# vision-agh/apse_uav

Hardware: AMD Instinct MI355X
Metric: 4K UAV frames/sec (whole node) (higher is better)
Workload: dtype f32

## Files before the change

apse_uav_amd/_lib.py:

```python
import ctypes as C
import os

import numpy as np

_HERE = os.path.dirname(os.path.abspath(__file__))
_TREE_LIB = os.path.join(_HERE, "libapse_hip.so")
LIB_PATH = os.environ.get("APSE_HIP_LIB") or _TREE_LIB
TOOL_ENTRIES = ("apse_winograd_pack_filter", "apse_winograd_conv2d")

APSE_OK = 0


class ApseError(RuntimeError):
    pass


class Config(C.Structure):
    _fields_ = [
        ("struct_size", C.c_int), ("device", C.c_int), ("max_batch", C.c_int),
        ("frame_h", C.c_int), ("frame_w", C.c_int), ("image_h", C.c_int), ("image_w", C.c_int),
        ("blocks", C.c_int * 4), ("num_classes", C.c_int),
        ("score_thresh", C.c_float), ("box_nms", C.c_float), ("rpn_nms", C.c_float), ("mask_thresh", C.c_float),
        ("rpn_pre_topk", C.c_int), ("rpn_post_topk", C.c_int), ("dets_per_image", C.c_int),
        ("pixel_mean", C.c_float * 3), ("assoc_roi", C.c_int), ("embed_dim", C.c_int), ("assoc_scale", C.c_float),
        ("compute_dtype", C.c_int), ("storage16", C.c_int),
    ]


class ConfigArch(Config):
    _fields_ = [("arch", C.c_int)]


class ResultsLayout(C.Structure):
    _fields_ = [("bytes", C.c_size_t), ("n_max", C.c_int), ("dets_per_image", C.c_int), ("embed_dim", C.c_int),
                ("max_batch", C.c_int)] + [(k, C.c_size_t) for k in (
                    "total", "offset", "prop_count", "img", "cls", "roi", "score", "box_resized", "box", "valid", "rect",
                    "mass", "centroid", "closest", "embedding")]


class RenderItem(C.Structure):
    _fields_ = [("image", C.c_int), ("rect", C.c_int * 4), ("words_per_row", C.c_int), ("bits", C.c_void_p),
                ("box", C.c_float * 4), ("rgb", C.c_uint8 * 4), ("label_off", C.c_int), ("label_len", C.c_int)]


class MotsWindow(C.Structure):
    _fields_ = [("rect", C.c_int * 4), ("words_per_row", C.c_int), ("area", C.c_int), ("bits", C.c_void_p)]


class MotsObject(C.Structure):
    _fields_ = [("rect", C.c_int * 4), ("words_per_row", C.c_int), ("score", C.c_float), ("bits", C.c_void_p)]


class ConvDesc(C.Structure):
    _fields_ = [(k, C.c_int) for k in ("B", "H", "W", "Cin", "Cout", "KH", "KW", "stride", "pad", "relu", "res_mode",
                                       "cfg", "splitk", "prec", "fuse_reduce", "x_st", "res_st", "y_st")]


_lib = None


def load():
    global _lib
    if _lib is not None:
        return _lib
    if not os.path.exists(LIB_PATH):
        raise ApseError("libapse_hip.so not found at %s: build it with `python -c 'import __graft_entry__ as g; g.build()'` "
                        "or `make -C apse_uav_amd/csrc` (there is no CPU fallback)" % LIB_PATH)
    import torch
    lib = C.CDLL(LIB_PATH)
    vp, i, f, sz = C.c_void_p, C.c_int, C.c_float, C.c_size_t
    sig = {
        "apse_create": ([C.POINTER(Config), C.POINTER(vp)], i),
        "apse_destroy": ([vp], None),
        "apse_last_error": ([vp], C.c_char_p),
        "apse_version": ([], C.c_char_p),
        "apse_set_weight": ([vp, C.c_char_p, vp, C.POINTER(C.c_int64), i], i),
        "apse_finalize_weights": ([vp], i),
        "apse_set_resize_tables": ([vp, vp, vp, i, vp, vp, i], i),
        "apse_set_camera": ([vp, C.POINTER(C.c_double), C.POINTER(C.c_double), i, vp, i, i], i),
        "apse_preprocess_frames": ([vp, vp, i, vp], i),
        "apse_preprocess_images": ([vp, vp, i, vp], i),
        "apse_backbone": ([vp, i, vp], i),
        "apse_rpn": ([vp, i, vp], i),
        "apse_rpn_levels": ([vp, i, i, vp], i),
        "apse_box_head": ([vp, i, vp], i),
        "apse_set_detections": ([vp, vp, vp, vp, vp, i, vp], i),
        "apse_mask_tail": ([vp, i, vp], i),
        "apse_embed": ([vp, i, vp], i),
        "apse_forward": ([vp, i, vp], i),
        "apse_results_describe": ([vp, C.POINTER(ResultsLayout)], i),
        "apse_read_results": ([vp, vp, sz, vp], i),
        "apse_read_results_begin": ([vp, vp, sz, vp], i),
        "apse_read_results_end": ([vp, vp], i),
        "apse_copy_mask_window": ([vp, i, i, i, i, i, vp, vp], i),
        "apse_copy_mask_windows": ([vp, i, vp, vp, vp, vp, vp], i),
        "apse_host_copy": ([vp, vp, sz, i], i),
        "apse_feature_shape": ([vp, C.c_char_p, C.POINTER(C.c_int * 3)], i),
        "apse_export_feature": ([vp, C.c_char_p, vp, i, vp], i),
        "apse_debug_tensor": ([vp, C.c_char_p, vp, sz, C.POINTER(sz), vp], i),
        "apse_flops": ([vp, i, C.c_double, C.c_double], C.c_double),
        "apse_profile": ([vp, i], i),
        "apse_profile_read": ([vp, C.POINTER(C.c_double * 42), i], i),
        "apse_conv_packed_elems": ([C.POINTER(ConvDesc)], sz),
        "apse_conv_pack_weight": ([C.POINTER(ConvDesc), vp, i, vp, vp], i),
        "apse_conv2d": ([C.POINTER(ConvDesc), vp, vp, vp, vp, vp, vp, sz, vp], i),
        "apse_winograd_pack_filter": ([vp, i, i, vp], i),
        "apse_winograd_conv2d": ([C.POINTER(ConvDesc), vp, vp, vp, vp, vp], i),
        "apse_maxpool3x3s2": ([vp, vp, i, i, i, i, vp], i),
        "apse_maxpool3x3s2_typed": ([vp, vp, i, i, i, i, i, vp], i),
        "apse_roi_align": ([C.POINTER(vp), C.POINTER(i), C.POINTER(i), vp, i, i, i, vp, vp], i),
        "apse_roi_align_typed": ([C.POINTER(vp), C.POINTER(i), C.POINTER(i), vp, i, i, i, i, vp, vp], i),
        "apse_roi_pool": ([vp, i, i, vp, vp, i, i, f, vp, vp], i),
        "apse_roi_features": ([vp, i, vp, vp, i, i, vp, vp], i),
        "apse_nms_rank": ([vp, vp, vp, i, i, i, i, f, i, vp, vp, vp, vp, vp], i),
        "apse_mask_centroid_dense": ([vp, i, i, C.POINTER(C.c_int * 3), vp], i),
        "apse_mask_closest_dense": ([vp, i, i, f, f, C.POINTER(C.c_int * 2), vp], i),
        "apse_l2_normalize": ([vp, vp, i, i, vp], i),
        "apse_sqdist": ([vp, vp, i, i, i, vp, vp], i),
        "apse_undistort_gamma": ([vp, vp, i, i, i, C.POINTER(C.c_double), C.POINTER(C.c_double), i, vp, i, i, vp], i),
        "apse_lab_tables_host": ([vp, vp, C.c_size_t], C.c_size_t),
        "apse_replay_create": ([i, i, f, i], vp),
        "apse_replay_destroy": ([vp], None),
        "apse_replay_step": ([vp, i, i, vp, vp, vp, C.c_char_p, i, vp], i),
        "apse_replay_packed": ([vp, vp, C.c_longlong, i, i, i, vp, C.c_longlong], C.c_longlong),
        "apse_replay_max_id": ([vp], i),
        "apse_replay_next_id": ([vp], i),
        "apse_render_workspace_bytes": ([i, i, i], sz),
        "apse_render_instances": ([vp, vp, i, i, i, i, vp, i, vp, sz, vp, i, vp, sz, vp], i),
        "apse_render_pack_mask": ([vp, i, i, vp, vp], i),
        "apse_render_font_host": ([vp, sz], sz),
        "apse_mots_split_workspace_bytes": ([], sz),
        "apse_mots_split_idmap": ([vp, i, i, i, vp, sz, vp, vp, vp, vp, sz, vp], i),
        "apse_mots_rle_to_bits": ([vp, vp, i, i, i, vp, vp], i),
        "apse_mots_overlaps": ([vp, i, vp, i, vp, i, vp, vp], i),
        "apse_mots_shift_overlaps": ([vp, i, vp, i, i, i, vp, vp], i),
        "apse_mots_render_idmap": ([vp, vp, i, i, i, vp, vp], i),
        "apse_resize_normalize": ([vp, vp, vp, vp, vp, vp, i, vp, vp, i, i, i, i, i, i, i, i, C.POINTER(f * 3), vp], i),
        "apse_assoc_fc_workspace_bytes": ([i, i, i], sz),
        "apse_assoc_fc_forward": ([vp, vp, vp, i, i, i, vp, vp, vp, sz, vp], i),
        "apse_assoc_fc_backward": ([vp, vp, vp, vp, i, i, i, vp, vp, vp, sz, vp], i),
        "apse_triplet_workspace_bytes": ([i], sz),
        "apse_triplet_hard_forward": ([vp, vp, i, i, f, i, vp, vp, sz, vp], i),
        "apse_triplet_all_forward": ([vp, vp, i, i, f, i, vp, vp, sz, vp], i),
        "apse_triplet_hard_backward": ([vp, i, i, i, vp, vp, vp, vp], i),
        "apse_triplet_all_backward": ([vp, i, i, i, vp, vp, vp, vp], i),
        "apse_sgd_step": ([vp, vp, vp, C.c_longlong, f, f, f, f, i, i, vp], i),
        "apse_coco_box_iou": ([vp, vp, vp, i, i, i, vp, vp, vp, vp, vp], i),
        "apse_coco_poly_to_bits": ([vp, vp, i, vp, i, vp, vp, vp, i, vp, vp, vp, vp], i),
        "apse_coco_match": ([vp, vp, vp, i, i, i, vp, vp, vp, i, vp, vp, vp, i, vp, i, vp, i, vp, vp, vp, vp, vp], i),
        "apse_coco_accumulate_workspace_bytes": ([C.c_longlong], sz),
        "apse_coco_sort_lists": ([vp, vp, i, vp, C.c_longlong, i, vp, vp, sz, vp], i),
        "apse_coco_accumulate": ([vp, vp, vp, i, vp, i, vp, vp, vp, C.c_longlong, i, vp, i, i, i, i, i, vp, vp, vp, vp, sz,
                                  vp], i),
        "apse_mask_roi_features": ([vp, i, vp, i, vp, vp], i),
        "apse_mask_train_workspace_bytes": ([i, i], sz),
        "apse_mask_pack_elems": ([i, i, i, i], sz),
        "apse_mask_pack_weight": ([vp, vp, i, i, i, i, i, vp, vp, vp], i),
        "apse_mask_conv_forward": ([vp, vp, vp, i, i, i, i, i, i, i, i, i, i, i, vp, vp, sz, vp], i),
        "apse_mask_conv3x3": ([vp, vp, vp, i, i, vp, vp], i),
        "apse_mask_relu_grad": ([vp, vp, C.c_longlong, vp, vp], i),
        "apse_mask_bias_grad": ([vp, C.c_longlong, vp, vp, sz, vp], i),
        "apse_mask_wgrad": ([vp, vp, i, i, vp, vp, sz, vp], i),
        "apse_mask_loss_forward": ([vp, i, vp, vp, i, vp, vp, sz, vp], i),
        "apse_mask_loss_backward": ([vp, i, vp, vp, i, vp, vp, vp], i),
        "apse_mask_predictor_backward": ([vp, vp, vp, vp, i, i, vp, vp, vp, vp, sz, vp], i),
        "apse_augment_u8": ([vp, i, i, i, vp, vp, vp, vp, vp], i),
    }
    for name, (args, ret) in sig.items():
        if name in TOOL_ENTRIES and LIB_PATH != _TREE_LIB and not hasattr(lib, name):
            continue
        fn = getattr(lib, name)
        fn.argtypes = args
        fn.restype = ret
    _lib = lib
    return lib


EXPORTS = ["apse_create", "apse_destroy", "apse_last_error", "apse_version", "apse_set_weight", "apse_finalize_weights",
           "apse_set_resize_tables", "apse_set_camera", "apse_preprocess_frames", "apse_preprocess_images", "apse_backbone", "apse_rpn", "apse_rpn_levels",
           "apse_box_head", "apse_set_detections", "apse_mask_tail", "apse_embed", "apse_forward", "apse_results_describe",
           "apse_read_results", "apse_read_results_begin", "apse_read_results_end", "apse_copy_mask_window", "apse_copy_mask_windows", "apse_host_copy", "apse_feature_shape", "apse_export_feature", "apse_debug_tensor",
           "apse_flops", "apse_profile", "apse_profile_read", "apse_conv_packed_elems", "apse_conv_pack_weight", "apse_conv2d", "apse_winograd_pack_filter", "apse_winograd_conv2d", "apse_maxpool3x3s2",
           "apse_maxpool3x3s2_typed", "apse_roi_align", "apse_roi_align_typed", "apse_roi_pool", "apse_roi_features", "apse_nms_rank", "apse_mask_centroid_dense", "apse_mask_closest_dense",
           "apse_l2_normalize", "apse_sqdist", "apse_undistort_gamma", "apse_lab_tables_host", "apse_resize_normalize", "apse_replay_create", "apse_replay_destroy",
           "apse_replay_step", "apse_replay_packed", "apse_replay_max_id", "apse_replay_next_id", "apse_render_workspace_bytes",
           "apse_render_instances", "apse_render_pack_mask", "apse_render_font_host", "apse_mots_split_workspace_bytes",
           "apse_mots_split_idmap", "apse_mots_rle_to_bits", "apse_mots_overlaps", "apse_mots_shift_overlaps", "apse_mots_render_idmap",
           "apse_assoc_fc_workspace_bytes", "apse_assoc_fc_forward", "apse_assoc_fc_backward", "apse_triplet_workspace_bytes",
           "apse_triplet_hard_forward", "apse_triplet_all_forward", "apse_triplet_hard_backward", "apse_triplet_all_backward",
           "apse_sgd_step", "apse_coco_box_iou", "apse_coco_poly_to_bits", "apse_coco_match",
           "apse_coco_accumulate_workspace_bytes", "apse_coco_sort_lists", "apse_coco_accumulate",
           "apse_mask_roi_features", "apse_mask_train_workspace_bytes", "apse_mask_pack_elems", "apse_mask_pack_weight",
           "apse_mask_conv_forward", "apse_mask_conv3x3", "apse_mask_relu_grad", "apse_mask_bias_grad", "apse_mask_wgrad", "apse_mask_loss_forward",
           "apse_mask_loss_backward", "apse_mask_predictor_backward", "apse_augment_u8"]


def stream_ptr():
    import torch
    return C.c_void_p(torch.cuda.current_stream().cuda_stream)


def check(rc, ctx=None, what=""):
    if rc != APSE_OK:
        msg = load().apse_last_error(ctx).decode() if ctx is not None else ""
        raise ApseError("%s failed (code %d) %s" % (what, rc, msg))


def ptr(t):
    if t is None:
        return C.c_void_p(0)
    if isinstance(t, np.ndarray):
        assert t.flags["C_CONTIGUOUS"]
        return C.c_void_p(t.ctypes.data)
    assert t.is_contiguous()
    return C.c_void_p(t.data_ptr())
```

apse_uav_amd/config.py:

```python
import copy
import os

import yaml


class CfgNode(dict):
    def __init__(self, init=None):
        super().__init__()
        self.__dict__["_frozen"] = False
        for k, v in (init or {}).items():
            self[k] = CfgNode(v) if isinstance(v, dict) else v

    def __getattr__(self, k):
        try:
            return self[k]
        except KeyError:
            raise AttributeError(k)

    def __setattr__(self, k, v):
        if self.__dict__.get("_frozen"):
            raise AttributeError("attempt to modify frozen CfgNode key %r" % k)
        self[k] = v

    def freeze(self):
        self.__dict__["_frozen"] = True
        for v in self.values():
            if isinstance(v, CfgNode):
                v.freeze()

    def defrost(self):
        self.__dict__["_frozen"] = False
        for v in self.values():
            if isinstance(v, CfgNode):
                v.defrost()

    def clone(self):
        c = CfgNode(copy.deepcopy(_plain(self)))
        return c

    def _merge(self, other):
        for k, v in other.items():
            if isinstance(v, dict) and isinstance(self.get(k), CfgNode):
                self[k]._merge(v)
            else:
                self[k] = CfgNode(v) if isinstance(v, dict) else (tuple(v) if isinstance(v, list) else v)

    def merge_from_file(self, path):
        data = _load_yaml_chain(path)
        if (data.get("MODEL", {}).get("ROI_HEADS", {}).get("NAME") == C4_ROI_HEADS and "MODEL" in self
                and not is_c4(self)):
            _apply_c4_defaults(self)
        self._merge(data)

    def merge_from_list(self, kv):
        for k, v in zip(kv[0::2], kv[1::2]):
            node = self
            parts = k.split(".")
            for p in parts[:-1]:
                node = node[p]
            node[parts[-1]] = v


def _deep_update(dst, src):
    for k, v in src.items():
        if isinstance(v, dict) and isinstance(dst.get(k), dict):
            _deep_update(dst[k], v)
        else:
            dst[k] = v
    return dst


def _load_yaml_chain(path):
    with open(path) as f:
        data = yaml.safe_load(f) or {}
    base = data.pop("_BASE_", None)
    if not base:
        return data
    if not os.path.isabs(base):
        base = os.path.join(os.path.dirname(path), base)
    return _deep_update(_load_yaml_chain(base), data)


def _plain(n):
    return {k: (_plain(v) if isinstance(v, CfgNode) else v) for k, v in n.items()}


def get_cfg():
    return CfgNode({
        "VERSION": 2,
        "MODEL": {
            "DEVICE": "cuda",
            "META_ARCHITECTURE": "GeneralizedRCNN",
            "WEIGHTS": "",
            "MASK_ON": True,
            "PIXEL_MEAN": (103.530, 116.280, 123.675),
            "PIXEL_STD": (1.0, 1.0, 1.0),
            "BACKBONE": {"NAME": "build_resnet_fpn_backbone"},
            "RESNETS": {"DEPTH": 101, "OUT_FEATURES": ("res2", "res3", "res4", "res5"),
                        "STRIDE_IN_1X1": True, "NORM": "FrozenBN", "RES2_OUT_CHANNELS": 256, "STEM_OUT_CHANNELS": 64},
            "FPN": {"IN_FEATURES": ("res2", "res3", "res4", "res5"), "OUT_CHANNELS": 256, "FUSE_TYPE": "sum", "NORM": ""},
            "ANCHOR_GENERATOR": {"SIZES": ((32,), (64,), (128,), (256,), (512,)),
                                 "ASPECT_RATIOS": ((0.5, 1.0, 2.0),), "OFFSET": 0.0},
            "RPN": {"IN_FEATURES": ("p2", "p3", "p4", "p5", "p6"), "PRE_NMS_TOPK_TEST": 1000,
                    "POST_NMS_TOPK_TEST": 1000, "NMS_THRESH": 0.7, "BBOX_REG_WEIGHTS": (1.0, 1.0, 1.0, 1.0),
                    "MIN_SIZE": 0},
            "ROI_HEADS": {"NAME": "StandardROIHeads", "IN_FEATURES": ("p2", "p3", "p4", "p5"), "NUM_CLASSES": 80,
                          "SCORE_THRESH_TEST": 0.05, "NMS_THRESH_TEST": 0.5},
            "ROI_BOX_HEAD": {"NAME": "FastRCNNConvFCHead", "NUM_FC": 2, "FC_DIM": 1024, "POOLER_RESOLUTION": 7,
                             "POOLER_SAMPLING_RATIO": 0, "POOLER_TYPE": "ROIAlignV2",
                             "BBOX_REG_WEIGHTS": (10.0, 10.0, 5.0, 5.0)},
            "ROI_MASK_HEAD": {"NAME": "MaskRCNNConvUpsampleHead", "NUM_CONV": 4, "CONV_DIM": 256,
                              "POOLER_RESOLUTION": 14, "POOLER_SAMPLING_RATIO": 0, "POOLER_TYPE": "ROIAlignV2"},
        },
        "INPUT": {"MIN_SIZE_TEST": 800, "MAX_SIZE_TEST": 1333, "FORMAT": "BGR", "MIN_SIZE_TRAIN": (800,), "MAX_SIZE_TRAIN": 1333,
                  "MIN_SIZE_TRAIN_SAMPLING": "choice"},
        "TEST": {"DETECTIONS_PER_IMAGE": 100},
        "DATASETS": {"TRAIN": ("coco_2017_train",), "TEST": ("coco_2017_val",)},
        "APSE": {"DTYPE": "f32", "MAX_BATCH": 1, "FUSED_PREPROC": True, "STORAGE16": True, "CONTEXT_CACHE": 1},
    })


C4_ROI_HEADS = "Res5ROIHeads"
C4_ANCHOR_SIZES = ((32, 64, 128, 256, 512),)
C4_ANCHOR_RATIOS = ((0.5, 1.0, 2.0),)


def is_c4(cfg):
    return cfg.MODEL.ROI_HEADS.NAME == C4_ROI_HEADS


def _apply_c4_defaults(cfg):
    m = cfg.MODEL
    m.BACKBONE.NAME = "build_resnet_backbone"
    m.RESNETS.OUT_FEATURES = ("res4",)
    m.RESNETS.RES5_DILATION = 1
    m.ANCHOR_GENERATOR.SIZES = C4_ANCHOR_SIZES
    m.ANCHOR_GENERATOR.ASPECT_RATIOS = C4_ANCHOR_RATIOS
    m.RPN.IN_FEATURES = ("res4",)
    m.RPN.PRE_NMS_TOPK_TEST = 6000
    m.RPN.POST_NMS_TOPK_TEST = 1000
    m.ROI_HEADS.NAME = C4_ROI_HEADS
    m.ROI_HEADS.IN_FEATURES = ("res4",)
    m.ROI_BOX_HEAD.NAME = ""
    m.ROI_BOX_HEAD.NUM_FC = 0
    m.ROI_BOX_HEAD.POOLER_RESOLUTION = 14
    m.ROI_MASK_HEAD.NUM_CONV = 0
    m.ROI_MASK_HEAD.POOLER_RESOLUTION = 14


def check_c4_supported(cfg):
    m = cfg.MODEL
    if tuple(tuple(s) for s in m.ANCHOR_GENERATOR.SIZES) != C4_ANCHOR_SIZES or \
            tuple(tuple(r) for r in m.ANCHOR_GENERATOR.ASPECT_RATIOS) != C4_ANCHOR_RATIOS or \
            float(m.ANCHOR_GENERATOR.get("OFFSET", 0.0)) != 0.0:
        raise ValueError("C4: only detectron2's default anchors are supported (sizes %s, ratios %s, offset 0)"
                         % (C4_ANCHOR_SIZES, C4_ANCHOR_RATIOS))
    if int(m.RESNETS.get("RES5_DILATION", 1)) != 1:
        raise ValueError("C4: RES5_DILATION 2 is not supported")
    if not m.MASK_ON:
        raise ValueError("C4: box-only models (MASK_ON False) are not supported")
    if tuple(m.RPN.IN_FEATURES) != ("res4",) or tuple(m.ROI_HEADS.IN_FEATURES) != ("res4",):
        raise ValueError("C4: the RPN and the ROI heads read res4")
    if int(m.ROI_BOX_HEAD.POOLER_RESOLUTION) != 14 or int(m.ROI_MASK_HEAD.POOLER_RESOLUTION) != 14 or \
            int(m.ROI_MASK_HEAD.NUM_CONV) != 0:
        raise ValueError("C4: pooler resolution 14 and no mask convolutions (NUM_CONV 0) are required")


CLASSES_NAMES = ["car", "truck", "bus", "person"]


def setup_cfg(weights="", score_thresh=0.5, num_classes=4, device="cuda", arch="FPN"):
    if arch not in ("FPN", "C4"):
        raise ValueError("arch must be 'FPN' or 'C4'")
    cfg = get_cfg()
    if arch == "C4":
        _apply_c4_defaults(cfg)
    cfg.MODEL.ROI_HEADS.SCORE_THRESH_TEST = score_thresh
    cfg.MODEL.ROI_HEADS.NUM_CLASSES = num_classes
    cfg.MODEL.WEIGHTS = weights
    cfg.MODEL.MASK_ON = True
    cfg.MODEL.DEVICE = device
    return cfg
```

apse_uav_amd/csrc/detector.hip:

```cpp
#include "detector_ctx.h"

#include <math.h>
#include <string.h>

static std::string g_create_error;

int fail(apse_ctx* c, int code, const std::string& msg) {
    if (c) c->err = msg; else g_create_error = msg;
    return code;
}
int apse_fail_global(int code, const char* msg) { return fail(nullptr, code, msg); }

static int take_event_pair(apse_ctx* c, hipStream_t s) {
    if (!c->prof_on) return -1;
    if (c->ev_used == 0) {
        hipEventRecord(c->ev_pool[c->ev_base], s);
        hipEventRecord(c->ev_pool[c->ev_base + 1], s);
        c->ev_used = 2;
    }
    if (c->ev_used + 2 > APSE_EV_HALF) return -1;
    const int e0 = c->ev_base + c->ev_used;
    c->ev_used += 2;
    return e0;
}

static int run_plan(apse_ctx* c, std::vector<Step>& plan, int batch, hipStream_t s) {
    int* total_dev = reinterpret_cast<int*>(c->res + c->lay.total);
    int* propcnt_dev = reinterpret_cast<int*>(c->res + c->lay.prop_count);
    for (size_t si = 0; si < plan.size(); ++si) {
        Step& st = plan[si];
        int rc = APSE_OK;
        if (st.kind == S_CONV) {
            ConvParams p = st.c.p;
            for (size_t sj = si + 1; sj < plan.size() && sj <= si + 2; ++sj)
                if (plan[sj].kind == S_CONV) {
                    const ConvParams& q = plan[sj].c.p;
                    const size_t elems = q.wu ? (size_t)16 * q.Cout * (1 << q.cin_log2) : (size_t)apse_roundup(q.Cout, 128) * q.KH * q.KWCp;
                    p.next_w = q.w16 ? (const void*)q.w16 : (q.wu ? (const void*)q.wu : (const void*)q.w);
                    const size_t bytes = elems * (q.w16 ? 2 : 4);
                    p.next_w_bytes = bytes > (64u << 20) ? (64u << 20) : (unsigned)bytes;
                    break;
                }
            p.B = st.c.fixed_items > 0 ? st.c.fixed_items : batch * st.c.b_mult;
            p.M = p.B * p.OH * p.OW;
            p.ws = c->ws;
            p.tile_cnt = nullptr;
            p.m_count = nullptr; p.m_per_item = p.OH * p.OW; p.m_hint = 0;
            int cfg = st.c.cfg;
            if (st.c.count_kind == 2) {
                p.m_count = total_dev;
                const int mh = (c->hint_total > 0 ? c->hint_total : 1) * p.m_per_item;
                p.m_hint = mh < p.M ? mh : p.M;
                if (p.prec != 0 && p.splitk == 1 && (cfg == 0 || cfg == 1 || cfg == 3)) {
                    int sk_dyn = 1;
                    const int cfg_dyn = apse_conv_pick_cfg(p.m_hint, p.Cout, p.steps_total, &sk_dyn);
                    if (sk_dyn == 1 && (cfg_dyn == 0 || cfg_dyn == 1 || cfg_dyn == 3)) cfg = cfg_dyn;
                }
            }
            else if (st.c.count_kind == 1 && batch == 1) p.m_count = propcnt_dev;
            const int e0 = take_event_pair(c, s);
            const hipEvent_t ev0 = e0 >= 0 ? c->ev_pool[e0] : nullptr, ev1 = e0 >= 0 ? c->ev_pool[e0 + 1] : nullptr;
            if (st.c.pool_y) {
                rc = apse_k_stem_pool16(p.x, p.w16, p.bias, st.c.pool_y, batch, p.H, p.W, p.prec, s, ev0, ev1);
                cfg = APSE_CFG_STEMPOOL;
            } else if (p.wu) {
                rc = apse_launch_conv_winograd(p, s, ev0, ev1);
            } else {
                rc = apse_launch_conv(p, cfg, s, ev0, ev1);
                cfg = apse_conv_effective_cfg(p, cfg);
            }
            if (e0 >= 0) c->pending.push_back({cfg, st.c.flops_per_item, st.c.count_kind, st.c.b_mult, batch, e0, e0 + 1});
        } else if (st.kind == S_BNECK) {
            const int e0 = take_event_pair(c, s);
            const ConvParams& q1 = st.c.p;
            rc = apse_k_bottleneck64_fused16(st.x, st.p3.res, st.y, q1.w16, q1.bias, st.p2.w16, st.p2.bias, st.p3.w16, st.p3.bias, batch,
                                             st.H, st.W, st.C, st.st, s, e0 >= 0 ? c->ev_pool[e0] : nullptr,
                                             e0 >= 0 ? c->ev_pool[e0 + 1] : nullptr);
            if (e0 >= 0) c->pending.push_back({APSE_CFG_BNECK, st.c.flops_per_item, 0, 1, batch, e0, e0 + 1});
        } else if (st.kind == S_MAXPOOL) {
            rc = apse_k_maxpool3x3s2(st.x, st.y, batch, st.H, st.W, st.C, st.st, s);
        } else {
            rc = apse_k_subsample2(st.x, st.y, batch, st.H, st.W, st.C, st.st, s);
        }
        if (rc != APSE_OK) return fail(c, rc, "launch failed at step " + st.c.name);
    }
    return APSE_OK;
}

int fill_camera(UndistortParams& p, int H, int W, const double* m, const double* dist, int ndist, int do_undistort, int do_gamma) {
    memset(&p, 0, sizeof p);
    if (!m || ndist > 14 || ndist < 0 || (ndist > 0 && !dist)) return APSE_E_INVALID;
    for (int i = 0; i < ndist && i < 12; ++i) p.k[i] = dist[i];
    if (ndist > 12 && (dist[12] != 0.0 || (ndist > 13 && dist[13] != 0.0))) return APSE_E_INVALID;
    const double a = m[0], b = m[1], c = m[2], dd = m[3], e = m[4], f = m[5], g = m[6], h = m[7], k = m[8];
    const double det = a * (e * k - f * h) - b * (dd * k - f * g) + c * (dd * h - e * g);
    if (det == 0.0) return APSE_E_INVALID;
    const double id = 1.0 / det;
    p.ir[0] = (e * k - f * h) * id; p.ir[1] = (c * h - b * k) * id; p.ir[2] = (b * f - c * e) * id;
    p.ir[3] = (f * g - dd * k) * id; p.ir[4] = (a * k - c * g) * id; p.ir[5] = (c * dd - a * f) * id;
    p.ir[6] = (dd * h - e * g) * id; p.ir[7] = (b * g - a * h) * id; p.ir[8] = (a * e - b * dd) * id;
    p.fx = m[0]; p.fy = m[4]; p.u0 = m[2]; p.v0 = m[5];
    p.H = H; p.W = W; p.do_undistort = do_undistort; p.do_gamma = do_gamma;
    return APSE_OK;
}

extern "C" {

#ifndef APSE_SRC_HASH
#define APSE_SRC_HASH "unknown"
#endif
const char* apse_version(void) { return "apse_hip 0.6 (gfx950, f32 / bf16 / f16 MFMA) src " APSE_SRC_HASH; }

int apse_create(const apse_config* cfg, apse_ctx** out) {
    if (!cfg || !out) return fail(nullptr, APSE_E_INVALID, "null argument");
    const int old_size = (int)offsetof(apse_config, arch);
    if (cfg->struct_size != (int)sizeof(apse_config) && cfg->struct_size != old_size)
        return fail(nullptr, APSE_E_INVALID, "apse_config size mismatch");
    apse_config cf;
    memset(&cf, 0, sizeof cf);
    memcpy(&cf, cfg, (size_t)cfg->struct_size);
    cf.struct_size = (int)sizeof(apse_config);
    cfg = &cf;
    if (cfg->arch != 0 && cfg->arch != 1) return fail(nullptr, APSE_E_INVALID, "arch must be 0 (FPN) or 1 (C4)");
    if (cfg->arch == 1) {
        if (cfg->rpn_pre_topk < 1 || cfg->rpn_pre_topk > APSE_C4_MAX_PRE_TOPK)
            return fail(nullptr, APSE_E_INVALID, "C4 (arch 1): rpn_pre_topk " + std::to_string(cfg->rpn_pre_topk) + " outside 1.." +
                                                 std::to_string(APSE_C4_MAX_PRE_TOPK));
        if (cfg->compute_dtype != 0)
            return fail(nullptr, APSE_E_INVALID, "C4 (arch 1): compute_dtype must be 0 (f32); the 16-bit modes are FPN only");
        if (cfg->max_batch > APSE_C4_MAX_BATCH)
            return fail(nullptr, APSE_E_INVALID, "C4 (arch 1): max_batch " + std::to_string(cfg->max_batch) + " above the limit " +
                                                 std::to_string(APSE_C4_MAX_BATCH));
    }
    const int pre_cap = cfg->arch == 1 ? APSE_C4_MAX_PRE_TOPK : 1000;
    if (cfg->max_batch < 1 || cfg->max_batch > 64 || cfg->rpn_pre_topk > pre_cap || cfg->rpn_post_topk > 1000 ||
        cfg->dets_per_image > 100 || cfg->num_classes < 1 || cfg->num_classes > APSE_MAX_CLASSES || cfg->embed_dim > 256 ||
        cfg->max_batch * cfg->dets_per_image > 1024)
        return fail(nullptr, APSE_E_INVALID, "config out of supported range");
    {
        const double t = cfg->score_thresh;
        const double per_roi = t > 0.0 ? ceil(1.0 / t) - 1.0 : (double)cfg->num_classes;
        const double bound = (double)cfg->rpn_post_topk * (per_roi < cfg->num_classes ? per_roi : (double)cfg->num_classes);
        if (bound >= 40000.0)
            return fail(nullptr, APSE_E_INVALID,
                        "box candidate bound rpn_post_topk * min(num_classes, ceil(1 / score_thresh) - 1) = " +
                            std::to_string((long long)bound) + " reaches 40000, where detectron2's batched_nms changes method");
    }
    if (cfg->frame_h < 1 || cfg->frame_w < 1 || cfg->frame_h > APSE_MAX_FRAME_H || cfg->frame_w > APSE_MAX_FRAME_W)
        return fail(nullptr, APSE_E_INVALID, "frame size out of supported range (1 <= frame_h <= " + std::to_string(APSE_MAX_FRAME_H) +
                                             ", 1 <= frame_w <= " + std::to_string(APSE_MAX_FRAME_W) + ")");
    if (cfg->compute_dtype < 0 || cfg->compute_dtype > 2 || (cfg->compute_dtype && !cfg->storage16))
        return fail(nullptr, APSE_E_INVALID, "compute_dtype 1 / 2 (bf16 / f16 matrix cores) needs storage16 = 1: the f32-storage variant "
                                             "of the 16-bit modes was removed in round 4 (no BASELINE configuration uses it)");
    int ndev = 0;
    if (hipGetDeviceCount(&ndev) != hipSuccess || ndev <= 0)
        return fail(nullptr, APSE_E_HIP, "no HIP device visible: the apse_uav hot path has no CPU fallback");
    if (hipSetDevice(cfg->device) != hipSuccess) return fail(nullptr, APSE_E_HIP, "hipSetDevice failed");
    apse_ctx* c = new apse_ctx();
    c->cfg = *cfg;
    c->c4 = cfg->arch == 1;
    {
        const char* e = getenv("APSE_F32_WINOGRAD");
        c->f32_winograd = !(e && atoi(e) == 0);
    }
    *out = c;
    return APSE_OK;
}

void apse_destroy(apse_ctx* c) {
    if (!c) return;
    hipSetDevice(c->cfg.device);
    for (void* p : c->allocs) hipFree(p);
    if (c->rf_mask) hipFree(c->rf_mask);
    if (c->mrf_idx) hipFree(c->mrf_idx);
    if (c->read_ev) hipEventDestroy(c->read_ev);
    for (int k = 0; k < 2; ++k) {
        if (c->given_ev[k]) hipEventDestroy(c->given_ev[k]);
        if (c->given_host[k]) hipHostFree(c->given_host[k]);
    }
    delete c;
}

const char* apse_last_error(apse_ctx* c) { return c ? c->err.c_str() : g_create_error.c_str(); }

int apse_set_weight(apse_ctx* c, const char* name, const float* host, const int64_t* shape, int ndim) {
    if (!c || !name || !host || !shape || ndim < 1 || ndim > 4) return fail(c, APSE_E_INVALID, "bad weight argument");
    if (c->finalized) return fail(c, APSE_E_STATE, "weights already finalized");
    HostW w;
    size_t n = 1;
    for (int i = 0; i < ndim; ++i) { w.shape.push_back(shape[i]); n *= (size_t)shape[i]; }
    w.v.assign(host, host + n);
    c->hw[name] = std::move(w);
    return APSE_OK;
}

int apse_finalize_weights(apse_ctx* c) {
    if (!c) return APSE_E_INVALID;
    if (c->finalized) return fail(c, APSE_E_STATE, "already finalized");
    hipSetDevice(c->cfg.device);
    int rc = c->c4 ? build_plan_c4(c) : build_plan(c);
    if (rc) return rc;
    c->hw.clear();
    c->finalized = true;
    return APSE_OK;
}

int apse_set_resize_tables(apse_ctx* c, const int* hb, const int* hc, int hk, const int* vb, const int* vc, int vk) {
    if (!c || !hb || !hc || !vb || !vc) return fail(c, APSE_E_INVALID, "null table");
    const apse_config& g = c->cfg;
    std::vector<int> a(hb, hb + 2 * g.image_w), b(hc, hc + (size_t)hk * g.image_w), d(vb, vb + 2 * g.image_h),
        e(vc, vc + (size_t)vk * g.image_h);
    for (int i = 0; i < g.image_w; ++i)
        if (a[2 * i] < 0 || a[2 * i + 1] > hk || a[2 * i] + a[2 * i + 1] > g.frame_w) return fail(c, APSE_E_INVALID, "bad horizontal bounds");
    for (int i = 0; i < g.image_h; ++i)
        if (d[2 * i] < 0 || d[2 * i + 1] > vk || d[2 * i] + d[2 * i + 1] > g.frame_h) return fail(c, APSE_E_INVALID, "bad vertical bounds");
    c->hb = dupload(c, a); c->hc = dupload(c, b); c->vb = dupload(c, d); c->vc = dupload(c, e);
    c->hk = hk; c->vk = vk;
    c->hcT = nullptr;
    if (hk <= 8) {
        std::vector<int> t((size_t)8 * g.image_w, 0);
        for (int i = 0; i < g.image_w; ++i)
            for (int j = 0; j < a[2 * i + 1] && j < hk; ++j) t[(size_t)j * g.image_w + i] = b[(size_t)i * hk + j];
        c->hcT = dupload(c, t);
    }
    return APSE_OK;
}

#define NEED_READY(c, batch)                                                                     \
    if (!(c) || !(c)->finalized) return fail(c, APSE_E_STATE, "weights not finalized");          \
    if ((batch) < 1 || (batch) > (c)->cfg.max_batch) return fail(c, APSE_E_INVALID, "batch out of range");

int apse_preprocess_frames(apse_ctx* c, const uint8_t* frames, int batch, void* stream) {
    NEED_READY(c, batch);
    if (!c->hb) return fail(c, APSE_E_STATE, "resize tables not set");
    const apse_config& g = c->cfg;
    int rc = apse_k_pil_resize(frames, c->rs_tmp, c->t["input"].p, c->t["input"].st, nullptr, c->hb, c->hc, c->hk, c->vb, c->vc, c->vk, batch,
                               g.frame_h, g.frame_w, g.image_h, g.image_w, c->PH, c->PW, g.pixel_mean, c->cam_on ? &c->cam : nullptr, c->cam_lut, c->cam_map_ok ? c->cam_map : nullptr,
                               c->hcT, c->rs_pitch, (hipStream_t)stream);
    return rc ? fail(c, rc, "pil resize launch failed") : APSE_OK;
}

int apse_preprocess_images(apse_ctx* c, const float* images, int batch, void* stream) {
    NEED_READY(c, batch);
    const apse_config& g = c->cfg;
    int rc = apse_k_chw_norm(images, c->t["input"].p, c->t["input"].st, batch, g.image_h, g.image_w, c->PH, c->PW, g.pixel_mean,
                             (hipStream_t)stream);
    return rc ? fail(c, rc, "chw normalise launch failed") : APSE_OK;
}

int apse_backbone(apse_ctx* c, int batch, void* stream) {
    NEED_READY(c, batch);
    return run_plan(c, c->backbone, batch, (hipStream_t)stream);
}

int apse_rpn_levels(apse_ctx* c, int batch, int level_mask, void* stream) {
    NEED_READY(c, batch);
    level_mask &= 31;
    if (!level_mask) return fail(c, APSE_E_INVALID, "empty RPN level mask");
    int first_level = 0;
    while (!((level_mask >> first_level) & 1)) ++first_level;
    hipStream_t s = (hipStream_t)stream;
    const apse_config& g = c->cfg;
    if (c->c4 && level_mask != 31) return fail(c, APSE_E_INVALID, "C4 (arch 1) has one RPN level: level_mask must be 31");
    int rc = run_plan(c, c->rpnhead, batch, s);
    if (rc) return rc;
    if (c->c4) {
        int* propcnt = reinterpret_cast<int*>(c->res + c->lay.prop_count);
        rc = apse_k_c4_rpn(&c->c4r, g.rpn_pre_topk, g.rpn_post_topk, (float)g.image_h, (float)g.image_w, (float)log(1000.0 / 16.0),
                           g.rpn_nms, c->dec_boxes, c->dec_scores, c->dec_valid, c->c4_nms, c->props, c->prop_scores, c->prop_entry,
                           propcnt, batch, s);
        c->box_maxc_clean = false;
        return rc ? fail(c, rc, "C4 rpn selection launch failed") : APSE_OK;
    }
    for (size_t i = 0; i < c->stages.size(); ++i) {
        rc = apse_k_rpn_topk_stage(c->rl_dev, c->stage_dev[i], (int)c->stages[i].size(), c->lists, c->nslots, batch,
                                   i == 0 ? c->maxc : nullptr, s);
        if (rc) return fail(c, rc, "rpn top-k stage launch failed");
    }
    rc = apse_k_rpn_decode(c->rl_dev, g.rpn_pre_topk, c->lists, c->nslots, c->final_slot_dev, (float)g.image_h, (float)g.image_w,
                           (float)log(1000.0 / 16.0), c->dec_boxes, c->dec_scores, c->dec_valid, c->maxc, level_mask, batch, s);
    if (rc) return fail(c, rc, "rpn decode launch failed");
    rc = apse_k_nms_percat(c->dec_boxes, c->dec_scores, c->dec_valid, 5 * g.rpn_pre_topk, g.rpn_pre_topk, 0, c->maxc, g.rpn_nms,
                           c->keep_idx, c->keep_cnt, 5, c->nms_scratch, first_level, batch, 1, s);
    if (rc) return fail(c, rc, "rpn nms launch failed");
    int* propcnt = reinterpret_cast<int*>(c->res + c->lay.prop_count);
    rc = apse_k_rank_final(c->dec_boxes, c->dec_scores, 5 * g.rpn_pre_topk, c->keep_idx, c->keep_cnt, 5, g.rpn_post_topk, c->props,
                           c->prop_scores, c->prop_entry, propcnt, c->maxc + g.max_batch, batch, s);
    c->box_maxc_clean = true;
    if (rc) return fail(c, rc, "rpn rank launch failed");
    return APSE_OK;
}

int apse_rpn(apse_ctx* c, int batch, void* stream) { return apse_rpn_levels(c, batch, 31, stream); }

static int pack_from_dets(apse_ctx* c, int batch, hipStream_t s) {
    const apse_config& g = c->cfg;
    uint8_t* r = c->res;
    c->sums_dirty = false;
    return apse_k_pack_detections(c->det_boxes, c->det_scores, c->det_entry, c->det_cnt, batch, g.dets_per_image, g.num_classes,
                                  (float*)(r + c->lay.box_resized), (float*)(r + c->lay.score), (int*)(r + c->lay.cls),
                                  (int*)(r + c->lay.img), (int*)(r + c->lay.roi), (int*)(r + c->lay.total),
                                  (int*)(r + c->lay.offset), c->sums, s);
}

int apse_box_head(apse_ctx* c, int batch, void* stream) {
    NEED_READY(c, batch);
    hipStream_t s = (hipStream_t)stream;
    const apse_config& g = c->cfg;
    int* propcnt = reinterpret_cast<int*>(c->res + c->lay.prop_count);
    const int P = g.rpn_post_topk, K = g.num_classes;
    int rc;
    if (c->c4) {
        const Tens& f = c->t["res4"];
        rc = apse_k_roi_align_c4(f.p, f.H, f.W, f.C, 1.0f / 16.0f, c->props, nullptr, propcnt, nullptr, P, batch * P, 14,
                                 c->t["box_pooled"].p, s);
        if (rc) return fail(c, rc, "C4 roi_align(14) launch failed");
        rc = run_plan(c, c->c4_res5box, batch, s);
        if (rc) return rc;
        const Tens& r5 = c->t["box_res5"];
        rc = apse_k_mean_cells(r5.p, batch * P, r5.H * r5.W, r5.C, c->t["box_mean"].p, s);
        if (rc) return fail(c, rc, "C4 mean launch failed");
    } else {
        rc = apse_k_roi_align(&c->fm, c->props, nullptr, propcnt, nullptr, P, batch * P, 7, c->t["box_pooled"].p,
                              c->t["box_pooled"].st, s);
        if (rc) return fail(c, rc, "roi_align(7) launch failed");
    }
    rc = run_plan(c, c->boxhead, batch, s);
    if (rc) return rc;
    const float wts[4] = {10.f, 10.f, 5.f, 5.f};
    if (!c->box_maxc_clean) hipMemsetAsync(c->maxc + g.max_batch, 0, sizeof(uint32_t) * g.max_batch, s);
    c->box_maxc_clean = false;
    if (c->wide) {
        rc = apse_k_box_candidates_wide(c->t["box_pred"].p, c->pred_ld, K, c->props, propcnt, P, (float)g.image_h, (float)g.image_w,
                                        g.score_thresh, wts, (float)log(1000.0 / 16.0), c->cand_boxes, c->cand_scores, c->cand_valid,
                                        c->maxc + g.max_batch, c->probs, c->cls_list, c->cls_cnt, batch, s);
        if (rc) return fail(c, rc, "box candidates (wide) launch failed");
        rc = apse_k_nms_lists(c->cand_boxes, c->cand_scores, P * K, c->cls_list, c->cls_cnt, P, c->maxc + g.max_batch, g.box_nms,
                              c->keep_idx, c->keep_cnt, K, c->nms_scratch, batch, s);
        if (rc) return fail(c, rc, "box nms (wide) launch failed");
        rc = apse_k_rank_wide(c->cand_boxes, c->cand_scores, P * K, c->keep_idx, c->keep_cnt, K, g.dets_per_image, c->det_boxes,
                              c->det_scores, c->det_entry, c->det_cnt, batch, s);
        if (rc) return fail(c, rc, "box rank (wide) launch failed");
        rc = pack_from_dets(c, batch, s);
        return rc ? fail(c, rc, "pack launch failed") : APSE_OK;
    }
    rc = apse_k_box_candidates(c->t["box_pred"].p, c->pred_ld, K, c->props, propcnt, P, (float)g.image_h, (float)g.image_w, g.score_thresh,
                               wts, (float)log(1000.0 / 16.0), c->cand_boxes, c->cand_scores, c->cand_valid,
                               c->maxc + g.max_batch, c->probs, batch, s);
    if (rc) return fail(c, rc, "box candidates launch failed");
    rc = apse_k_nms_percat(c->cand_boxes, c->cand_scores, c->cand_valid, P * K, 0, K, c->maxc + g.max_batch, g.box_nms, c->keep_idx,
                           c->keep_cnt, K, c->nms_scratch, 0, batch, 0, s);
    if (rc) return fail(c, rc, "box nms launch failed");
    rc = apse_k_rank_final(c->cand_boxes, c->cand_scores, P * K, c->keep_idx, c->keep_cnt, K, g.dets_per_image, c->det_boxes,
                           c->det_scores, c->det_entry, c->det_cnt, nullptr, batch, s);
    if (rc) return fail(c, rc, "box rank launch failed");
    rc = pack_from_dets(c, batch, s);
    return rc ? fail(c, rc, "pack launch failed") : APSE_OK;
}

int apse_set_detections(apse_ctx* c, const float* boxes, const int* classes, const float* scores, const int* counts, int batch,
                        void* stream) {
    NEED_READY(c, batch);
    hipStream_t s = (hipStream_t)stream;
    const apse_config& g = c->cfg;
    const int KD = g.dets_per_image, K = g.num_classes;
    const size_t nb = (size_t)g.max_batch * KD;
    const size_t bytes = nb * 16 + nb * 4 + nb * 4 + (size_t)g.max_batch * 4;
    const int slot = c->given_k ^= 1;
    if (!c->given_host[slot]) {
        HIPCHK(c, hipHostMalloc((void**)&c->given_host[slot], bytes, hipHostMallocDefault));
        HIPCHK(c, hipEventCreateWithFlags(&c->given_ev[slot], hipEventDisableTiming));
    } else {
        HIPCHK(c, hipEventSynchronize(c->given_ev[slot]));
    }
    float* db = (float*)c->given_host[slot];
    float* ds = db + nb * 4;
    int* de = (int*)(ds + nb);
    int* dc = de + nb;
    memset(db, 0, nb * 16 + nb * 4);
    for (size_t i = 0; i < nb; ++i) de[i] = -1;
    for (int b = 0; b < g.max_batch; ++b) dc[b] = 0;
    int o = 0;
    for (int b = 0; b < batch; ++b) {
        if (counts[b] < 0 || counts[b] > KD) return fail(c, APSE_E_INVALID, "too many given detections");
        dc[b] = counts[b];
        for (int k = 0; k < counts[b]; ++k, ++o) {
            memcpy(&db[((size_t)b * KD + k) * 4], boxes + (size_t)o * 4, 16);
            ds[(size_t)b * KD + k] = scores ? scores[o] : 1.0f;
            if (classes[o] < 0 || classes[o] >= K) return fail(c, APSE_E_INVALID, "class out of range");
            de[(size_t)b * KD + k] = k * K + classes[o];
        }
    }
    const size_t nbb = (size_t)batch * KD;
    HIPCHK(c, hipMemcpyAsync(c->det_boxes, db, nbb * 16, hipMemcpyHostToDevice, s));
    HIPCHK(c, hipMemcpyAsync(c->det_scores, ds, nbb * 4, hipMemcpyHostToDevice, s));
    HIPCHK(c, hipMemcpyAsync(c->det_entry, de, nbb * 4, hipMemcpyHostToDevice, s));
    HIPCHK(c, hipMemcpyAsync(c->det_cnt, dc, (size_t)batch * 4, hipMemcpyHostToDevice, s));
    HIPCHK(c, hipEventRecord(c->given_ev[slot], s));
    int rc = pack_from_dets(c, batch, s);
    return rc ? fail(c, rc, "pack launch failed") : APSE_OK;
}

int apse_mask_tail(apse_ctx* c, int batch, void* stream) {
    NEED_READY(c, batch);
    hipStream_t s = (hipStream_t)stream;
    const apse_config& g = c->cfg;
    uint8_t* r = c->res;
    const int NM = batch * g.dets_per_image;
    int* total = (int*)(r + c->lay.total);
    int rc;
    if (c->c4) {
        const Tens& f = c->t["res4"];
        rc = apse_k_roi_align_c4(f.p, f.H, f.W, f.C, 1.0f / 16.0f, (float*)(r + c->lay.box_resized), (int*)(r + c->lay.img), nullptr,
                                 total, 0, NM, 14, c->t["mask_pooled"].p, s);
    } else {
        rc = apse_k_roi_align(&c->fm, (float*)(r + c->lay.box_resized), (int*)(r + c->lay.img), nullptr, total, 0, NM, 14,
                              c->t["mask_pooled"].p, c->t["mask_pooled"].st, s);
    }
    if (rc) return fail(c, rc, "roi_align(14) launch failed");
    rc = run_plan(c, c->maskhead, batch, s);
    if (rc) return rc;
    PasteParams p;
    p.boxes = (float*)(r + c->lay.box_resized); p.cls = (int*)(r + c->lay.cls); p.total = total;
    p.logits = c->t["mask_logits"].p; p.M = c->t["mask_logits"].H; p.ldc = c->t["mask_logits"].C;
    p.sx = (float)((double)g.frame_w / (double)g.image_w); p.sy = (float)((double)g.frame_h / (double)g.image_h);
    p.out_h = g.frame_h; p.out_w = g.frame_w; p.words_per_row = c->wpr; p.thresh = g.mask_thresh;
    p.boxes_out = (float*)(r + c->lay.box); p.valid = (int*)(r + c->lay.valid); p.rect = (int*)(r + c->lay.rect);
    if (c->sums_dirty) HIPCHK(c, hipMemsetAsync(c->sums, 0, (size_t)g.max_batch * g.dets_per_image * 3 * sizeof(unsigned long long), s));
    c->sums_dirty = true;
    c->bits_cur ^= 1;
    if (!c->read_pending) c->bits_read = c->bits_cur;
    uint64_t* bits = c->bits2[c->bits_cur];
    p.bits = bits; p.sums = c->sums;
    unsigned long long* keys = (unsigned long long*)(r + c->lay.closest);
    rc = apse_k_mask_paste(&p, NM, keys, g.dets_per_image, s);
    if (rc) return fail(c, rc, "mask paste launch failed");
    rc = apse_k_closest_points(bits, p.rect, p.valid, c->sums, (int*)(r + c->lay.img), (int*)(r + c->lay.offset), total, NM,
                               g.dets_per_image, g.frame_h, g.frame_w, c->wpr, (int*)(r + c->lay.centroid), (int*)(r + c->lay.mass),
                               keys, c->hint_total, s);
    return rc ? fail(c, rc, "closest points launch failed") : APSE_OK;
}

int apse_embed(apse_ctx* c, int batch, void* stream) {
    NEED_READY(c, batch);
    hipStream_t s = (hipStream_t)stream;
    const apse_config& g = c->cfg;
    uint8_t* r = c->res;
    const int NM = batch * g.dets_per_image;
    int* total = (int*)(r + c->lay.total);
    int rc;
    if (c->c4) {
        const Tens& f = c->t["res4"];
        rc = apse_k_roi_pool_c4(f.p, f.H, f.W, f.C, (float*)(r + c->lay.box), (int*)(r + c->lay.img), total, NM, g.assoc_roi,
                                g.assoc_scale, (float*)c->t["assoc_pooled"].p, s);
    } else {
        const Tens& p2 = c->t["p2"];
        rc = apse_k_roi_pool(p2.p, p2.st, p2.H, p2.W, (float*)(r + c->lay.box), (int*)(r + c->lay.img), total, NM, g.assoc_roi,
                             g.assoc_scale, (float*)c->t["assoc_pooled"].p, 0, 0, s);
    }
    if (rc) return fail(c, rc, "roi_pool launch failed");
    if (c->ws_assoc) {
        const ConvParams& fp = c->embedfc[0].c.p;
        rc = apse_k_assoc_fc((const float*)c->t["assoc_pooled"].p, fp.w, fp.bias, c->ws_assoc, total, NM, fp.KH * fp.KWCp, g.embed_dim,
                             c->emb_raw, (float*)(r + c->lay.embedding), s);
        return rc ? fail(c, rc, "association FC launch failed") : APSE_OK;
    }
    rc = run_plan(c, c->embedfc, batch, s);
    if (rc) return rc;
    rc = apse_k_l2_normalize(c->emb_raw, (float*)(r + c->lay.embedding), g.embed_dim, total, NM, s);
    return rc ? fail(c, rc, "l2 normalise launch failed") : APSE_OK;
}

int apse_forward(apse_ctx* c, int batch, void* stream) {
    int rc;
    if ((rc = apse_backbone(c, batch, stream))) return rc;
    if ((rc = apse_rpn(c, batch, stream))) return rc;
    if ((rc = apse_box_head(c, batch, stream))) return rc;
    if ((rc = apse_mask_tail(c, batch, stream))) return rc;
    return apse_embed(c, batch, stream);
}

int apse_results_describe(apse_ctx* c, apse_results_layout* out) {
    if (!c || !out || !c->finalized) return fail(c, APSE_E_STATE, "not finalized");
    *out = c->lay;
    return APSE_OK;
}

int apse_read_results_begin(apse_ctx* c, void* host_dst, size_t bytes, void* stream) {
    if (!c || !c->finalized) return fail(c, APSE_E_STATE, "not finalized");
    if (bytes < c->lay.bytes) return fail(c, APSE_E_INVALID, "results buffer too small");
    if (!c->read_ev) HIPCHK(c, hipEventCreateWithFlags(&c->read_ev, hipEventDisableTiming));
    HIPCHK(c, hipMemcpyAsync(host_dst, c->res, c->lay.bytes, hipMemcpyDeviceToHost, (hipStream_t)stream));
    HIPCHK(c, hipEventRecord(c->read_ev, (hipStream_t)stream));
    c->read_pending = host_dst;
    c->bits_read = c->bits_cur;
    if (c->prof_on) {
        c->pending_read.swap(c->pending);
        c->pending.clear();
        c->cal_read = c->ev_used >= 2 ? c->ev_base : -1;
        c->ev_base ^= APSE_EV_HALF;
        c->ev_used = 0;
    }
    return APSE_OK;
}

int apse_read_results_end(apse_ctx* c, void* host_dst) {
    if (!c || !c->finalized) return fail(c, APSE_E_STATE, "not finalized");
    if (!c->read_pending || c->read_pending != host_dst) return fail(c, APSE_E_STATE, "apse_read_results_end without a matching _begin");
    HIPCHK(c, hipEventSynchronize(c->read_ev));
    c->read_pending = nullptr;
    c->hint_total = *reinterpret_cast<const int*>(reinterpret_cast<const uint8_t*>(host_dst) + c->lay.total);
    {
        uint8_t* h = reinterpret_cast<uint8_t*>(host_dst) + c->lay.closest;
        const int kd = c->cfg.dets_per_image, W = c->cfg.frame_w;
        int live = c->hint_total < 0 ? 0 : c->hint_total;
        if (live > c->lay.n_max) live = c->lay.n_max;
        for (size_t t = 0; t < (size_t)c->lay.n_max * kd; ++t) {
            unsigned long long k;
            memcpy(&k, h + 8 * t, 8);
            int xy[2] = {-1, -1};
            if (t < (size_t)live * kd && k != ~0ull) {
                const unsigned lin = (unsigned)(k & 0xffffffffu);
                xy[0] = (int)(lin % (unsigned)W) + 1; xy[1] = (int)(lin / (unsigned)W) + 1;
            }
            memcpy(h + 8 * t, xy, 8);
        }
    }
    if (c->prof_on) {
        const uint8_t* h = reinterpret_cast<const uint8_t*>(host_dst);
        const int total = *reinterpret_cast<const int*>(h + c->lay.total);
        const int* pc = reinterpret_cast<const int*>(h + c->lay.prop_count);
        float cal = 0.f;
        if (c->cal_read >= 0 && hipEventElapsedTime(&cal, c->ev_pool[c->cal_read], c->ev_pool[c->cal_read + 1]) != hipSuccess) cal = 0.f;
        for (auto& q : c->pending_read) {
            float ms = 0.f;
            if (hipEventElapsedTime(&ms, c->ev_pool[q.e0], c->ev_pool[q.e1]) != hipSuccess) continue;
            ms = ms > cal ? ms - cal : ms;
            double items = q.batch;
            if (q.count_kind == 1) { items = 0; for (int b = 0; b < q.batch; ++b) items += pc[b]; }
            else if (q.count_kind == 2) items = total;
            c->prof[q.cfg][0] += ms; c->prof[q.cfg][1] += q.flops_per_item * items; c->prof[q.cfg][2] += 1;
        }
        c->pending_read.clear();
        c->cal_read = -1;
    }
    return APSE_OK;
}

int apse_read_results(apse_ctx* c, void* host_dst, size_t bytes, void* stream) {
    int rc = apse_read_results_begin(c, host_dst, bytes, stream);
    return rc ? rc : apse_read_results_end(c, host_dst);
}

int apse_profile(apse_ctx* c, int enable) {
    if (!c) return APSE_E_INVALID;
    if (enable && c->ev_pool.empty()) {
        c->ev_pool.resize(2 * APSE_EV_HALF);
        for (auto& e : c->ev_pool) if (hipEventCreate(&e) != hipSuccess) return fail(c, APSE_E_HIP, "hipEventCreate");
    }
    c->prof_on = enable != 0;
    c->pending.clear();
    c->pending_read.clear();
    c->cal_read = -1;
    c->ev_used = 0;
    return APSE_OK;
}

int apse_profile_read(apse_ctx* c, double* out42, int reset) {
    if (!c || !out42) return APSE_E_INVALID;
    memcpy(out42, c->prof, sizeof(c->prof));
    if (reset) memset(c->prof, 0, sizeof(c->prof));
    return APSE_OK;
}

int apse_copy_mask_window(apse_ctx* c, int det, int x0, int y0, int x1, int y1, uint64_t* dst, void* stream) {
    if (!c || !c->finalized) return fail(c, APSE_E_STATE, "not finalized");
    const apse_config& g = c->cfg;
    if (det < 0 || det >= g.max_batch * g.dets_per_image || x0 < 0 || y0 < 0 || x1 > g.frame_w || y1 > g.frame_h || x1 <= x0 || y1 <= y0)
        return fail(c, APSE_E_INVALID, "bad mask window");
    const int w0 = x0 >> 6, w1 = (x1 + 63) >> 6;
    const uint64_t* src = c->bits2[c->bits_read] + ((size_t)det * g.frame_h + y0) * c->wpr + w0;
    HIPCHK(c, hipMemcpy2DAsync(dst, (size_t)(w1 - w0) * 8, src, (size_t)c->wpr * 8, (size_t)(w1 - w0) * 8, (size_t)(y1 - y0),
                               hipMemcpyDeviceToDevice, (hipStream_t)stream));
    return APSE_OK;
}

int apse_copy_mask_windows(apse_ctx* c, int n, const int* dets, const int* rects, uint64_t* dst, const long long* dst_off, void* stream) {
    if (!c || !c->finalized) return fail(c, APSE_E_STATE, "not finalized");
    const apse_config& g = c->cfg;
    if (n < 0 || n > 100 || (n > 0 && (!dets || !rects || !dst || !dst_off))) return fail(c, APSE_E_INVALID, "bad mask windows");
    long long src[100]; int nw[100], rows[100];
    for (int k = 0; k < n; ++k) {
        const int x0 = rects[k * 4], y0 = rects[k * 4 + 1], x1 = rects[k * 4 + 2], y1 = rects[k * 4 + 3];
        if (dets[k] < 0 || dets[k] >= g.max_batch * g.dets_per_image || x0 < 0 || y0 < 0 || x1 > g.frame_w || y1 > g.frame_h || x1 <= x0 ||
            y1 <= y0 || dst_off[k] < 0)
            return fail(c, APSE_E_INVALID, "bad mask window");
        const int w0 = x0 >> 6, w1 = (x1 + 63) >> 6;
        src[k] = ((long long)dets[k] * g.frame_h + y0) * c->wpr + w0;
        nw[k] = w1 - w0; rows[k] = y1 - y0;
    }
    int rc = apse_k_copy_mask_windows(c->bits2[c->bits_read], dst, n, src, dst_off, nw, rows, c->wpr, (hipStream_t)stream);
    return rc ? fail(c, rc, "mask windows launch failed") : APSE_OK;
}

int apse_feature_shape(apse_ctx* c, const char* name, int* chw3) {
    if (!c || !c->finalized) return fail(c, APSE_E_STATE, "not finalized");
    auto it = c->t.find(name);
    if (it == c->t.end()) return fail(c, APSE_E_MISSING, std::string("no tensor ") + name);
    chw3[0] = it->second.C; chw3[1] = it->second.H; chw3[2] = it->second.W;
    return APSE_OK;
}

int apse_export_feature(apse_ctx* c, const char* name, float* dst, int batch, void* stream) {
    NEED_READY(c, batch);
    auto it = c->t.find(name);
    if (it == c->t.end()) return fail(c, APSE_E_MISSING, std::string("no tensor ") + name);
    const Tens& t = it->second;
    int rc = apse_k_nhwc_to_nchw(t.p, dst, batch, t.H * t.W, t.C, t.st, (hipStream_t)stream);
    return rc ? fail(c, rc, "export launch failed") : APSE_OK;
}

int apse_roi_features(apse_ctx* c, int image, const float* rois, const uint8_t* masks, int n, int roi_size, float* out, void* stream) {
    if (!c || !c->finalized) return fail(c, APSE_E_STATE, "not finalized");
    const apse_config& g = c->cfg;
    if (image < 0 || image >= g.max_batch || n < 0 || roi_size < 1 || roi_size > 32 || (n > 0 && (!rois || !out)))
        return fail(c, APSE_E_INVALID, "bad roi_features arguments");
    if (c->c4) return fail(c, APSE_E_INVALID, "apse_roi_features reads p2: not available under C4 (arch 1)");
    if (n == 0) return APSE_OK;
    hipStream_t s = (hipStream_t)stream;
    const Tens& p2 = c->t["p2"];
    const float scale = (float)p2.W / (float)g.frame_w;
    int rc;
    if (!masks) {
        rc = apse_k_roi_pool(p2.p, p2.st, p2.H, p2.W, rois, nullptr, nullptr, n, roi_size, scale, out, image, 1, s);
        return rc ? fail(c, rc, "roi_pool launch failed") : APSE_OK;
    }
    const size_t need = (size_t)n * p2.H * p2.W;
    if (need > c->rf_mask_floats) {
        HIPCHK(c, hipStreamSynchronize(s));
        if (c->rf_mask) hipFree(c->rf_mask);
        c->rf_mask = nullptr; c->rf_mask_floats = 0;
        if (hipMalloc(reinterpret_cast<void**>(&c->rf_mask), need * sizeof(float)) != hipSuccess) return fail(c, APSE_E_NOMEM, "roi_features scratch");
        c->rf_mask_floats = need;
    }
    rc = apse_k_mask_resize(masks, n, g.frame_h, g.frame_w, p2.H, p2.W, c->rf_mask, s);
    if (rc) return fail(c, rc, "mask resize launch failed");
    rc = apse_k_roi_align_masked(p2.p, p2.st, p2.H, p2.W, image, rois, c->rf_mask, n, roi_size, 4, scale, out, s);
    return rc ? fail(c, rc, "masked roi_align launch failed") : APSE_OK;
}

int apse_mask_roi_features(apse_ctx* c, int image, const float* rois, int n, float* out, void* stream) {
    if (!c || !c->finalized) return fail(c, APSE_E_STATE, "not finalized");
    const apse_config& g = c->cfg;
    if (image < 0 || image >= g.max_batch || n < 0 || n > (1 << 20) || (n > 0 && (!rois || !out)))
        return fail(c, APSE_E_INVALID, "bad mask_roi_features arguments (image inside the batch, 0 <= n <= 2^20)");
    if (c->c4) return fail(c, APSE_E_INVALID, "apse_mask_roi_features pools p2..p5: not available under C4 (arch 1)");
    if (n == 0) return APSE_OK;
    hipStream_t s = (hipStream_t)stream;
    if ((size_t)n + 1 > c->mrf_cap) {
        HIPCHK(c, hipStreamSynchronize(s));
        if (c->mrf_idx) hipFree(c->mrf_idx);
        c->mrf_idx = nullptr; c->mrf_cap = 0;
        if (hipMalloc(reinterpret_cast<void**>(&c->mrf_idx), ((size_t)n + 1) * sizeof(int)) != hipSuccess) return fail(c, APSE_E_NOMEM, "mask_roi_features scratch");
        c->mrf_cap = (size_t)n + 1;
    }
    FpnMaps fm = c->fm;
    for (int l = 0; l < 4; ++l)
        fm.p[l] = reinterpret_cast<const char*>(fm.p[l]) + (size_t)image * fm.H[l] * fm.W[l] * 256 * (fm.st ? 2 : 4);
    int rc = apse_k_mask_roi_index(c->mrf_idx, n, s);
    if (rc) return fail(c, rc, "mask_roi_features index launch failed");
    rc = apse_k_roi_align(&fm, rois, c->mrf_idx, nullptr, c->mrf_idx + n, 0, n, 14, out, 0, s);
    return rc ? fail(c, rc, "roi_align(14) launch failed") : APSE_OK;
}

int apse_debug_tensor(apse_ctx* c, const char* name, void* dst, size_t max_bytes, size_t* bytes, void* stream) {
    if (!c || !c->finalized) return fail(c, APSE_E_STATE, "not finalized");
    const apse_config& g = c->cfg;
    const void* src = nullptr;
    size_t n = 0;
    const std::string nm = name;
    const int B = g.max_batch;
    if (nm == "proposals") { src = c->props; n = (size_t)B * g.rpn_post_topk * 16; }
    else if (nm == "proposal_scores") { src = c->prop_scores; n = (size_t)B * g.rpn_post_topk * 4; }
    else if (nm == "proposal_entry") { src = c->prop_entry; n = (size_t)B * g.rpn_post_topk * 4; }
    else if (nm == "rpn_decoded") { src = c->dec_boxes; n = (size_t)B * (c->c4 ? 1 : 5) * g.rpn_pre_topk * 16; }
    else if (nm == "rpn_decoded_scores") { src = c->dec_scores; n = (size_t)B * (c->c4 ? 1 : 5) * g.rpn_pre_topk * 4; }
    else if (nm == "rpn_decoded_valid") { src = c->dec_valid; n = (size_t)B * (c->c4 ? 1 : 5) * g.rpn_pre_topk * 4; }
    else if (nm == "box_probs") { src = c->probs; n = (size_t)B * g.rpn_post_topk * (g.num_classes + 1) * 4; }
    else if (nm == "cand_boxes") { src = c->cand_boxes; n = (size_t)B * g.rpn_post_topk * g.num_classes * 16; }
    else if (nm == "det_boxes") { src = c->det_boxes; n = (size_t)B * g.dets_per_image * 16; }
    else if (nm == "det_scores") { src = c->det_scores; n = (size_t)B * g.dets_per_image * 4; }
    else if (nm == "det_entry") { src = c->det_entry; n = (size_t)B * g.dets_per_image * 4; }
    else if (nm == "det_count") { src = c->det_cnt; n = (size_t)B * 4; }
    else if (nm == "embedding_raw") { src = c->emb_raw; n = (size_t)B * g.dets_per_image * g.embed_dim * 4; }
    else {
        auto it = c->t.find(nm);
        if (it == c->t.end()) return fail(c, APSE_E_MISSING, "no tensor " + nm);
        const Tens& t = it->second;
        int items = B;
        if (nm == "box_pooled" || nm == "box_fc1" || nm == "box_fc2" || nm == "box_pred" || nm == "box_mean" || nm == "box_res5")
            items = B * g.rpn_post_topk;
        else if (nm.rfind("mask_", 0) == 0 || nm.rfind("assoc_", 0) == 0) items = B * g.dets_per_image;
        src = t.p; n = (size_t)items * t.H * t.W * t.C * (t.st ? 2 : 4);
    }
    if (bytes) *bytes = n;
    if (!dst) return APSE_OK;
    if (n > max_bytes) return fail(c, APSE_E_INVALID, "debug buffer too small for " + nm);
    HIPCHK(c, hipMemcpyAsync(dst, src, n, hipMemcpyDeviceToDevice, (hipStream_t)stream));
    return APSE_OK;
}

double apse_flops(apse_ctx* c, int batch, double proposals, double detections) {
    if (!c || !c->finalized) return 0.0;
    double f = 0;
    for (auto& s : c->backbone) if (s.kind == S_CONV || s.kind == S_BNECK) f += s.c.flops_per_item * batch;
    for (auto& s : c->rpnhead) f += s.c.flops_per_item * batch;
    for (auto& s : c->c4_res5box) f += s.c.flops_per_item * proposals;
    for (auto& s : c->boxhead) f += s.c.flops_per_item * proposals;
    for (auto& s : c->maskhead) f += s.c.flops_per_item * detections;
    for (auto& s : c->embedfc) f += s.c.flops_per_item * detections;
    return f;
}

int apse_set_camera(apse_ctx* c, const double* m, const double* dist, int ndist, const uint8_t* lut_host, int do_undistort, int do_gamma) {
    if (!c) return APSE_E_INVALID;
    if (!do_undistort && !do_gamma) { c->cam_on = false; return APSE_OK; }
    if (do_gamma && !lut_host) return fail(c, APSE_E_INVALID, "gamma needs a 256-entry LUT");
    UndistortParams p;
    int rc = fill_camera(p, c->cfg.frame_h, c->cfg.frame_w, m, dist, ndist, do_undistort, do_gamma);
    if (rc) return fail(c, rc, "bad camera parameters (3x3 matrix, <= 14 distortion coefficients, tilt terms zero)");
    hipSetDevice(c->cfg.device);
    if (!c->cam_lut) {
        c->cam_lut = dalloc<LabTables>(c, 1);
        if (!c->cam_lut) return fail(c, APSE_E_NOMEM, "camera Lab tables alloc");
    }
    if (lut_host) {
        LabTables host;
        lab_tables_build(&host, lut_host);
        HIPCHK(c, hipDeviceSynchronize());
        HIPCHK(c, hipMemcpy(c->cam_lut, &host, sizeof(LabTables), hipMemcpyHostToDevice));
    }
    c->cam_map_ok = false;
    if (do_undistort) {
        if (!c->cam_map) {
            c->cam_map = dalloc<uint32_t>(c, (size_t)c->cfg.frame_h * c->cfg.frame_w + 4, false);
            if (!c->cam_map) return fail(c, APSE_E_NOMEM, "camera map alloc");
        }
        int* ovf = reinterpret_cast<int*>(reinterpret_cast<uint32_t*>(c->cam_map) + (size_t)c->cfg.frame_h * c->cfg.frame_w);
        HIPCHK(c, hipMemset(ovf, 0, sizeof(int)));
        rc = apse_k_undistort_build_map_compact(&p, c->cam_map, ovf, nullptr);
        if (rc) return fail(c, rc, "camera map launch failed");
        int overflow = 0;
        HIPCHK(c, hipMemcpy(&overflow, ovf, sizeof(int), hipMemcpyDeviceToHost));
        c->cam_map_ok = overflow == 0;
    }
    HIPCHK(c, hipDeviceSynchronize());
    c->cam = p;
    c->cam_on = true;
    return APSE_OK;
}

}
```

apse_uav_amd/csrc/detector_ctx.h:

```cpp
#pragma once
#include "apse_kernels.h"
#include "../../include/apse_hip.h"
#include "preproc_pixel.h"

#include <map>
#include <string>
#include <vector>

#define APSE_NARROW_CLASSES 6
#define APSE_EV_HALF 1024

struct HostW { std::vector<float> v; std::vector<int64_t> shape; };
struct Tens { float* p = nullptr; int H = 0, W = 0, C = 0; int st = 0; };

struct ConvStep {
    ConvParams p;
    int b_mult = 1;
    int fixed_items = 0;
    int cfg = 0;
    double flops_per_item = 0;
    int count_kind = 0;
    void* pool_y = nullptr;
    std::string name;
};
enum StepKind { S_CONV, S_MAXPOOL, S_SUBSAMPLE, S_BNECK };
struct Step { StepKind kind; ConvStep c; const float* x; float* y; int H, W, C; int st = 0; ConvParams p2, p3; };

struct apse_ctx {
    apse_config cfg;
    std::string err;
    bool f32_winograd = true;
    std::map<std::string, HostW> hw;
    bool finalized = false;
    int PH = 0, PW = 0;
    std::vector<void*> allocs;
    std::map<std::string, Tens> t;
    std::vector<Step> backbone, rpnhead, boxhead, maskhead, embedfc;
    float* ws = nullptr; size_t ws_floats = 0; int* tile_cnt = nullptr;
    int *hb = nullptr, *hc = nullptr, *vb = nullptr, *vc = nullptr; int hk = 0, vk = 0; uint8_t* rs_tmp = nullptr;
    int rs_pitch = 0;
    int* hcT = nullptr;
    RpnLevels rl_host; RpnLevels* rl_dev = nullptr;
    std::vector<std::vector<TopkJob>> stages; std::vector<TopkJob*> stage_dev; int nslots = 0; uint64_t* lists = nullptr;
    int final_slot_host[5]; int* final_slot_dev = nullptr;
    float *dec_boxes = nullptr, *dec_scores = nullptr; int* dec_valid = nullptr; uint32_t* maxc = nullptr;
    int *keep_idx = nullptr, *keep_cnt = nullptr; void* nms_scratch = nullptr;
    float *props = nullptr, *prop_scores = nullptr; int *prop_entry = nullptr;
    FpnMaps fm;
    float *cand_boxes = nullptr, *cand_scores = nullptr, *probs = nullptr; int* cand_valid = nullptr;
    int pred_ld = 32;
    bool wide = false;
    int *cls_list = nullptr, *cls_cnt = nullptr;
    float *det_boxes = nullptr, *det_scores = nullptr; int *det_entry = nullptr, *det_cnt = nullptr;
    apse_results_layout lay; uint8_t* res = nullptr;
    uint64_t* bits2[2] = {nullptr, nullptr}; int bits_cur = 0, bits_read = 0;
    unsigned long long* sums = nullptr; int wpr = 0; bool sums_dirty = false;
    float* emb_raw = nullptr;
    float* ws_assoc = nullptr;
    float* rf_mask = nullptr; size_t rf_mask_floats = 0;
    int* mrf_idx = nullptr; size_t mrf_cap = 0;
    bool box_maxc_clean = false;
    UndistortParams cam; bool cam_on = false; LabTables* cam_lut = nullptr; void* cam_map = nullptr; bool cam_map_ok = false;
    int hint_total = 8;
    hipEvent_t read_ev = nullptr; void* read_pending = nullptr;
    uint8_t* given_host[2] = {nullptr, nullptr}; hipEvent_t given_ev[2] = {nullptr, nullptr}; int given_k = 0;
    bool prof_on = false; std::vector<hipEvent_t> ev_pool; int ev_used = 0;
    struct Pending { int cfg; double flops_per_item; int count_kind; int b_mult; int batch; int e0, e1; };
    std::vector<Pending> pending; double prof[APSE_NCFG][3] = {{0}};
    int ev_base = 0, cal_read = -1; std::vector<Pending> pending_read;
    uint64_t* op_bits = nullptr; unsigned long long* op_sums = nullptr; size_t op_bits_words = 0;
    bool c4 = false;
    C4Rpn c4r; void* c4_nms = nullptr;
    std::vector<Step> c4_res5box;
};

int fail(apse_ctx* c, int code, const std::string& msg);
#define HIPCHK(c, call)                                                                        \
    do {                                                                                       \
        hipError_t e_ = (call);                                                                \
        if (e_ != hipSuccess) return fail(c, APSE_E_HIP, std::string(#call) + ": " + hipGetErrorString(e_)); \
    } while (0)

template <typename T>
static T* dalloc(apse_ctx* c, size_t n, bool zero = true) {
    void* p = nullptr;
    if (hipMalloc(&p, n * sizeof(T) > 0 ? n * sizeof(T) : 16) != hipSuccess) return nullptr;
    if (zero) hipMemset(p, 0, n * sizeof(T));
    c->allocs.push_back(p);
    return reinterpret_cast<T*>(p);
}
template <typename T>
static T* dupload(apse_ctx* c, const std::vector<T>& v) {
    T* p = dalloc<T>(c, v.size(), false);
    if (p && !v.empty()) hipMemcpy(p, v.data(), v.size() * sizeof(T), hipMemcpyHostToDevice);
    return p;
}

static inline int pow2_at_least(int v) { int p = 4; while (p < v) p <<= 1; return p; }
void pack_oihw(const float* w, int Cout, int Cin, int KH, int KW, int cin_p, const float* scale, float* out, int KWCp);
std::vector<float> winograd_filters(const float* oihw, int Cout, int Cin, int cin_p);
int build_plan(apse_ctx* c);
int build_plan_c4(apse_ctx* c);
int fill_camera(UndistortParams& p, int H, int W, const double* m, const double* dist, int ndist, int do_undistort, int do_gamma);
```

apse_uav_amd/csrc/plan.hip:

```cpp
#include "detector_ctx.h"

#include <math.h>
#include <stdio.h>
#include <string.h>

#define APSE_WINO_MIN_BLOCKS 128
#define APSE_EXPECTED_DETS 8

void pack_oihw(const float* w, int Cout, int Cin, int KH, int KW, int cin_p, const float* scale, float* out, int KWCp) {
    for (int o = 0; o < Cout; ++o) {
        const float sc = scale ? scale[o] : 1.0f;
        for (int r = 0; r < KH; ++r)
            for (int s = 0; s < KW; ++s)
                for (int ci = 0; ci < Cin; ++ci)
                    out[((size_t)o * KH + r) * KWCp + s * cin_p + ci] = w[(((size_t)o * Cin + ci) * KH + r) * KW + s] * sc;
    }
}

static const HostW* getw(apse_ctx* c, const std::string& n) {
    auto it = c->hw.find(n);
    return it == c->hw.end() ? nullptr : &it->second;
}

static Tens make_t(apse_ctx* c, const std::string& name, int items, int H, int W, int C, int st = 0) {
    Tens t;
    t.H = H; t.W = W; t.C = C; t.st = st;
    const size_t elems = (size_t)items * H * W * C;
    t.p = dalloc<float>(c, st ? (elems + 1) / 2 : elems);
    c->t[name] = t;
    return t;
}

struct ConvSpec {
    std::string name; std::vector<std::string> wnames;
    int KH, KW, stride, pad, relu;
    int fc_h = 0, fc_w = 0;
    int deconv = 0;
    int s2d = 0;
    std::string out_name;
    int items = 1;
    const Tens* res = nullptr; int res_mode = 0;
    int y_ld = 0;
    int count_kind = 0;
    float* out_ptr = nullptr;
    const Tens* out_view = nullptr;
};

static uint16_t round16(float v, int dtype) {
    if (dtype == 2) {
        const _Float16 hval = (_Float16)v;
        uint16_t r;
        memcpy(&r, &hval, 2);
        return r;
    }
    uint32_t b;
    memcpy(&b, &v, 4);
    if ((b & 0x7fffffffu) > 0x7f800000u) return (uint16_t)((b >> 16) | 0x40);
    return (uint16_t)((b + 0x7fffu + ((b >> 16) & 1u)) >> 16);
}
static int storage_type(const apse_ctx* c) { return (c->cfg.compute_dtype >= 1 && c->cfg.storage16) ? c->cfg.compute_dtype : 0; }

static bool winograd_layer(const std::string& n) {
    return n == "backbone.fpn_output2" || n == "backbone.fpn_output3" || n == "rpn_t2" || n == "rpn_t3";
}
std::vector<float> winograd_filters(const float* oihw, int Cout, int Cin, int cin_p) {
    static const double G[4][3] = {{1, 0, 0}, {0.5, 0.5, 0.5}, {0.5, -0.5, 0.5}, {0, 0, 1}};
    std::vector<float> u((size_t)16 * Cout * cin_p, 0.f);
    for (int o = 0; o < Cout; ++o)
        for (int ci = 0; ci < Cin; ++ci) {
            const float* g = oihw + ((size_t)o * Cin + ci) * 9;
            double t[4][3];
            for (int i = 0; i < 4; ++i)
                for (int s = 0; s < 3; ++s) t[i][s] = G[i][0] * g[s] + G[i][1] * g[3 + s] + G[i][2] * g[6 + s];
            for (int i = 0; i < 4; ++i)
                for (int j = 0; j < 4; ++j) {
                    const double v = t[i][0] * G[j][0] + t[i][1] * G[j][1] + t[i][2] * G[j][2];
                    u[(((size_t)(ci / 8) * 16 + 4 * i + j) * Cout + o) * 8 + (ci & 7)] = (float)v;
                }
        }
    return u;
}

static int add_conv(apse_ctx* c, std::vector<Step>& plan, const ConvSpec& sp, const Tens& in, Tens* out) {
    const std::string& out_name = sp.out_name.empty() ? sp.name : sp.out_name;
    std::vector<float> rows;
    std::vector<float> bias;
    int Cout = 0, Cin = 0;
    const int KH = sp.KH, KW = sp.KW;
    for (const auto& wn : sp.wnames) {
        const HostW* w = getw(c, wn + ".weight");
        if (!w) return fail(c, APSE_E_MISSING, "missing weight " + wn + ".weight");
        int co, ci;
        std::vector<float> oihw;
        if (sp.fc_h > 0) {
            co = (int)w->shape[0];
            const int flat = (int)w->shape[1];
            ci = flat / (sp.fc_h * sp.fc_w);
            oihw = w->v;
        } else if (sp.deconv) {
            ci = (int)w->shape[0];
            const int cc = (int)w->shape[1];
            co = 4 * cc;
            oihw.assign((size_t)co * ci, 0.f);
            for (int i = 0; i < ci; ++i)
                for (int o = 0; o < cc; ++o)
                    for (int dy = 0; dy < 2; ++dy)
                        for (int dx = 0; dx < 2; ++dx)
                            oihw[((size_t)((dy * 2 + dx) * cc + o)) * ci + i] = w->v[(((size_t)i * cc + o) * 2 + dy) * 2 + dx];
        } else if (w->shape.size() == 2) {
            co = (int)w->shape[0]; ci = (int)w->shape[1]; oihw = w->v;
        } else if (sp.s2d) {
            if (w->shape.size() != 4 || w->shape[2] != 7 || w->shape[3] != 7 || w->shape[1] != 3 || KH != 4 || KW != 4)
                return fail(c, APSE_E_INVALID, "space-to-depth stem needs a 7x7 filter over 3 channels: " + wn);
            co = (int)w->shape[0]; ci = 12;
            oihw.assign((size_t)co * 12 * 16, 0.f);
            for (int o = 0; o < co; ++o)
                for (int ch = 0; ch < 3; ++ch)
                    for (int r = 0; r < 4; ++r)
                        for (int sx = 0; sx < 4; ++sx)
                            for (int dy = 0; dy < 2; ++dy)
                                for (int dx = 0; dx < 2; ++dx) {
                                    const int ky = 2 * r + dy - 1, kx = 2 * sx + dx - 1;
                                    if (ky < 0 || ky > 6 || kx < 0 || kx > 6) continue;
                                    oihw[(((size_t)o * 12 + (dy * 2 + dx) * 3 + ch) * 4 + r) * 4 + sx] = w->v[(((size_t)o * 3 + ch) * 7 + ky) * 7 + kx];
                                }
        } else {
            co = (int)w->shape[0]; ci = (int)w->shape[1]; oihw = w->v;
            if ((int)w->shape[2] != KH || (int)w->shape[3] != KW) return fail(c, APSE_E_INVALID, "kernel size mismatch " + wn);
        }
        if (Cin && ci != Cin) return fail(c, APSE_E_INVALID, "Cin mismatch in fused conv " + sp.name);
        Cin = ci;
        const HostW* g = getw(c, wn + ".norm.weight");
        std::vector<float> scale;
        const int nb = sp.deconv ? co / 4 : co;
        std::vector<float> b(nb, 0.f);
        if (g) {
            const HostW* be = getw(c, wn + ".norm.bias");
            const HostW* mu = getw(c, wn + ".norm.running_mean");
            const HostW* var = getw(c, wn + ".norm.running_var");
            if (!be || !mu || !var) return fail(c, APSE_E_MISSING, "incomplete norm for " + wn);
            scale.resize(co);
            for (int o = 0; o < co; ++o) {
                scale[o] = g->v[o] * (1.0f / sqrtf(var->v[o] + 1e-5f));
                b[o] = be->v[o] - mu->v[o] * scale[o];
            }
            const size_t per = (size_t)ci * KH * KW;
            for (int o = 0; o < co; ++o)
                for (size_t k = 0; k < per; ++k) oihw[(size_t)o * per + k] *= scale[o];
        } else {
            const HostW* bw = getw(c, wn + ".bias");
            if (bw) for (int o = 0; o < nb; ++o) b[o] = bw->v[o];
        }
        rows.insert(rows.end(), oihw.begin(), oihw.end());
        bias.insert(bias.end(), b.begin(), b.end());
        Cout += co;
    }
    const int cin_p = in.C;
    if (pow2_at_least(Cin) != cin_p && Cin != cin_p) return fail(c, APSE_E_INVALID, "input channels mismatch at " + sp.name);
    if (sp.s2d && (in.C != 16 || sp.stride != 1 || sp.pad != 2)) return fail(c, APSE_E_INVALID, "space-to-depth stem geometry");
    const int KWC = KW * cin_p, KWCp = apse_roundup(KWC, 32);
    const int Cout_p = apse_roundup(Cout, 128);
    std::vector<float> packed((size_t)Cout_p * KH * KWCp, 0.f);
    pack_oihw(rows.data(), Cout, Cin, KH, KW, cin_p, nullptr, packed.data(), KWCp);
    std::vector<float> bias_p(Cout_p, 0.f);
    for (size_t i = 0; i < bias.size(); ++i) bias_p[i] = bias[i];
    const bool use_bf16 = (c->cfg.compute_dtype >= 1 && Cout > 32 && sp.name != "assoc_fc" && sp.name != "box_pred" &&
                           sp.name != "mask_logits");
    float* wd = nullptr;
    uint16_t* wd16 = nullptr;
    if (use_bf16) {
        std::vector<uint16_t> p16(packed.size());
        for (size_t i = 0; i < packed.size(); ++i) p16[i] = round16(packed[i], c->cfg.compute_dtype);
        wd16 = dupload(c, p16);
    } else {
        wd = dupload(c, packed);
    }
    float* bd = dupload(c, bias_p);
    if ((!wd && !wd16) || !bd) return fail(c, APSE_E_NOMEM, "weight upload failed at " + sp.name);

    Step st;
    st.kind = S_CONV;
    ConvStep& cs = st.c;
    memset(&cs.p, 0, sizeof(cs.p));
    cs.name = sp.name;
    cs.b_mult = sp.items;
    cs.count_kind = sp.count_kind;
    ConvParams& p = cs.p;
    p.x = in.p; p.w = wd; p.w16 = wd16; p.bias = bd; p.res = sp.res ? sp.res->p : nullptr; p.res_mode = sp.res_mode;
    p.x_st = in.st; p.res_st = sp.res ? sp.res->st : 0;
    p.H = in.H; p.W = in.W; p.cin_log2 = apse_ilog2(cin_p);
    p.KH = KH; p.KW = KW; p.stride = sp.stride; p.pad = sp.pad; p.KWCp = KWCp;
    p.OH = (in.H + 2 * sp.pad - KH) / sp.stride + 1;
    p.OW = (in.W + 2 * sp.pad - KW) / sp.stride + 1;
    if (sp.s2d) { p.OH = in.H; p.OW = in.W; }
    p.Cout = Cout; p.relu = sp.relu;
    p.steps_total = KH * (KWCp / 32);
    p.splitk = 1;
    p.out_mode = sp.deconv ? 1 : 0;
    p.prec = use_bf16 ? c->cfg.compute_dtype : 0;
    p.cdec = sp.deconv ? Cout / 4 : 0;
    const int out_c = sp.deconv ? Cout / 4 : (sp.y_ld > 0 ? sp.y_ld : Cout);
    const int oh = sp.deconv ? 2 * p.OH : p.OH, ow = sp.deconv ? 2 * p.OW : p.OW;
    const int out_st = sp.out_view ? sp.out_view->st : ((use_bf16 && !sp.out_ptr) ? storage_type(c) : 0);
    if (out_st && (out_c & 7)) return fail(c, APSE_E_INVALID, "16-bit tensors need C % 8 == 0 at " + sp.name);
    Tens o;
    if (sp.out_view) { o = *sp.out_view; o.H = oh; o.W = ow; o.C = out_c; c->t[out_name] = o; }
    else if (sp.out_ptr) { o.p = sp.out_ptr; o.H = oh; o.W = ow; o.C = out_c; }
    else o = make_t(c, out_name, c->cfg.max_batch * sp.items, oh, ow, out_c, out_st);
    p.y_st = o.st;
    if (!o.p) return fail(c, APSE_E_NOMEM, "activation alloc failed at " + sp.name);
    p.y = o.p; p.y_ld = out_c; p.y_coff = 0;
    cs.flops_per_item = sp.s2d ? 2.0 * p.OH * p.OW * (double)Cout * 7 * 7 * 3
                               : 2.0 * p.OH * p.OW * (double)Cout * KH * KW * Cin;
    const int Mfull = c->cfg.max_batch * sp.items * p.OH * p.OW;
    int sk = 1;
    cs.cfg = apse_conv_pick_cfg(Mfull, Cout, p.steps_total, &sk);
    if (sp.count_kind == 2) {
        const int kd = c->cfg.dets_per_image < APSE_EXPECTED_DETS ? c->cfg.dets_per_image : APSE_EXPECTED_DETS;
        const int rows = kd * c->cfg.max_batch * p.OH * p.OW;
        sk = 1;
        cs.cfg = apse_conv_pick_cfg(rows < Mfull ? rows : Mfull, Cout, p.steps_total, &sk);
    }
    p.splitk = sk;
    if (sk > 1) {
        const size_t need = (size_t)sk * Mfull * Cout;
        if (need > c->ws_floats) c->ws_floats = need;
    }
    if (c->f32_winograd && winograd_layer(sp.name) && sp.count_kind == 0 && apse_conv_winograd_ok(p, c->cfg.max_batch * sp.items) &&
        apse_conv_winograd_blocks(p) >= APSE_WINO_MIN_BLOCKS) {
        p.wu = dupload(c, winograd_filters(rows.data(), Cout, Cin, cin_p));
        if (!p.wu) return fail(c, APSE_E_NOMEM, "weight upload failed at " + sp.name);
    }
    if (out) *out = o;
    plan.push_back(st);
    return APSE_OK;
}

static void layout_results(apse_ctx* c) {
    apse_results_layout& L = c->lay;
    memset(&L, 0, sizeof(L));
    const int B = c->cfg.max_batch, kd = c->cfg.dets_per_image, n = B * kd, E = c->cfg.embed_dim;
    L.n_max = n; L.dets_per_image = kd; L.embed_dim = E; L.max_batch = B;
    size_t o = 0;
    auto take = [&](size_t bytes) { size_t r = o; o += (bytes + 15) / 16 * 16; return r; };
    L.total = take(4);
    L.offset = take(4 * (B + 1));
    L.prop_count = take(4 * B);
    L.img = take(4 * n); L.cls = take(4 * n); L.roi = take(4 * n); L.score = take(4 * n);
    L.box_resized = take(16 * n); L.box = take(16 * n); L.valid = take(4 * n); L.rect = take(16 * n);
    L.mass = take(4 * n); L.centroid = take(8 * n);
    L.closest = take((size_t)8 * n * kd);
    L.embedding = take((size_t)4 * n * E);
    L.bytes = o;
}

static void alloc_box_inference(apse_ctx* c) {
    const apse_config& g = c->cfg;
    const int B = g.max_batch, POST = g.rpn_post_topk, K = g.num_classes, KD = g.dets_per_image;
    c->wide = K > APSE_NARROW_CLASSES;
    if (c->wide) {
        c->cls_list = dalloc<int>(c, (size_t)B * K * POST, false);
        c->cls_cnt = dalloc<int>(c, (size_t)B * K);
    }
    c->cand_boxes = dalloc<float>(c, (size_t)B * POST * K * 4);
    c->cand_scores = dalloc<float>(c, (size_t)B * POST * K);
    c->cand_valid = dalloc<int>(c, (size_t)B * POST * K);
    c->probs = dalloc<float>(c, (size_t)B * POST * (K + 1));
    c->det_boxes = dalloc<float>(c, (size_t)B * KD * 4);
    c->det_scores = dalloc<float>(c, (size_t)B * KD);
    c->det_entry = dalloc<int>(c, (size_t)B * KD);
    c->det_cnt = dalloc<int>(c, (size_t)B);
}

static int alloc_proposals(apse_ctx* c, int levels) {
    const apse_config& g = c->cfg;
    const int B = g.max_batch, PRE = g.rpn_pre_topk, POST = g.rpn_post_topk, K = g.num_classes;
    c->dec_boxes = dalloc<float>(c, (size_t)B * levels * PRE * 4);
    c->dec_scores = dalloc<float>(c, (size_t)B * levels * PRE);
    c->dec_valid = dalloc<int>(c, (size_t)B * levels * PRE);
    c->maxc = dalloc<uint32_t>(c, (size_t)2 * B);
    if (c->c4) c->c4_nms = dalloc<uint8_t>(c, apse_c4_nms_scratch_bytes(B), false);
    const int ncat = K > 8 ? K : 8;
    c->keep_idx = dalloc<int>(c, (size_t)B * ncat * APSE_NMS_SLOT);
    c->keep_cnt = dalloc<int>(c, (size_t)B * ncat);
    c->nms_scratch = dalloc<uint8_t>(c, apse_nms_scratch_bytes(ncat * B));
    c->props = dalloc<float>(c, (size_t)B * POST * 4);
    c->prop_scores = dalloc<float>(c, (size_t)B * POST);
    c->prop_entry = dalloc<int>(c, (size_t)B * POST);
    if (!c->dec_boxes || !c->dec_scores || !c->dec_valid || !c->maxc || (c->c4 && !c->c4_nms) || !c->keep_idx || !c->keep_cnt ||
        !c->nms_scratch || !c->props || !c->prop_scores || !c->prop_entry)
        return fail(c, APSE_E_NOMEM, c->c4 ? "C4 proposal buffers" : "proposal buffers");
    return APSE_OK;
}

static int finish_plan(apse_ctx* c, int feat_C) {
    const apse_config& g = c->cfg;
    const int B = g.max_batch, KD = g.dets_per_image, NM = B * KD;
    int rc;
    c->wpr = (g.frame_w + 63) / 64;
    for (int k = 0; k < 2; ++k) c->bits2[k] = dalloc<uint64_t>(c, (size_t)NM * g.frame_h * c->wpr, false);
    c->sums = dalloc<unsigned long long>(c, (size_t)NM * 3);
    if (!c->bits2[0] || !c->bits2[1]) return fail(c, APSE_E_NOMEM, "mask bit planes alloc");
    const int R = g.assoc_roi;
    Tens ap = make_t(c, "assoc_pooled", NM, R, R, feat_C);
    Tens er;
    {
        ConvSpec sp{"assoc_fc", {"association.fc"}, R, R, 1, 0, 0, R, R};
        c->emb_raw = dalloc<float>(c, (size_t)NM * g.embed_dim);
        sp.items = KD; sp.count_kind = 2; sp.out_ptr = c->emb_raw;
        rc = add_conv(c, c->embedfc, sp, ap, &er);
        if (rc) return rc;
        const ConvParams& fp = c->embedfc[0].c.p;
        if (fp.w && fp.KWCp == R * feat_C && apse_assoc_fc_ok(fp.KH * fp.KWCp, g.embed_dim) && !getenv("APSE_NO_ASSOC_FC")) {
            c->ws_assoc = dalloc<float>(c, (size_t)(fp.KH * fp.KWCp / 128) * NM * g.embed_dim, false);
            if (!c->ws_assoc) return fail(c, APSE_E_NOMEM, "association FC workspace");
        }
    }
    if (c->ws_floats) {
        c->ws = dalloc<float>(c, c->ws_floats, false);
        if (!c->ws) return fail(c, APSE_E_NOMEM, "split-K workspace alloc");
    }
    c->tile_cnt = dalloc<int>(c, 65536);
    c->rs_pitch = (g.image_w * 3 + 15) & ~15;
    c->rs_tmp = dalloc<uint8_t>(c, (size_t)B * g.frame_h * c->rs_pitch, false);
    hipError_t e = hipDeviceSynchronize();
    if (e != hipSuccess) return fail(c, APSE_E_HIP, std::string("plan build: ") + hipGetErrorString(e));
    return APSE_OK;
}

static int add_bottleneck(apse_ctx* c, std::vector<Step>& plan, const std::string& wp, const std::string& tp, const Tens& in, int items,
                          int stride, int count_kind, const std::string& out_name, Tens* out) {
    auto spec = [&](const char* part, int k, int s, int relu) {
        ConvSpec sp{tp + part, {wp + part}, k, k, s, k / 2, relu};
        sp.items = items; sp.count_kind = count_kind;
        return sp;
    };
    Tens sc, a, b2;
    const Tens* resp = &in;
    int rc;
    if (getw(c, wp + ".shortcut.weight")) {
        if ((rc = add_conv(c, plan, spec(".shortcut", 1, stride, 0), in, &sc))) return rc;
        resp = &sc;
    }
    if ((rc = add_conv(c, plan, spec(".conv1", 1, stride, 1), in, &a))) return rc;
    if ((rc = add_conv(c, plan, spec(".conv2", 3, 1, 1), a, &b2))) return rc;
    ConvSpec sp3 = spec(".conv3", 1, 1, 1);
    sp3.out_name = out_name; sp3.res = resp; sp3.res_mode = 1;
    return add_conv(c, plan, sp3, b2, out);
}

static void fuse_bottleneck16(apse_ctx* c, std::vector<Step>& plan, const std::string& name, const Tens& in, const Tens& out) {
    const size_t n = plan.size();
    const ConvParams &q1 = plan[n - 3].c.p, &q2 = plan[n - 2].c.p, &q3 = plan[n - 1].c.p;
    const int st16 = storage_type(c);
    if (!(st16 && q1.stride == 1 && q1.Cout == 64 && out.C == 256 && (in.C == 64 || in.C == 256) && q1.w16 && q2.w16 && q3.w16 &&
          q1.x_st == st16 && q1.y_st == st16 && q2.y_st == st16 && q3.y_st == st16 && q3.res_st == st16 && q2.KWCp == 192 &&
          q1.KWCp == in.C && q3.KWCp == 64 && (size_t)c->cfg.max_batch * in.H * in.W * in.C * 2 < 0xfffffff0ull &&
          !getenv("APSE_NO_BNECK_FUSE")))
        return;
    Step fs;
    fs.kind = S_BNECK;
    fs.c = plan[n - 3].c;
    fs.c.name = name;
    fs.c.flops_per_item = plan[n - 3].c.flops_per_item + plan[n - 2].c.flops_per_item + plan[n - 1].c.flops_per_item;
    fs.p2 = q2; fs.p3 = q3;
    fs.x = in.p; fs.y = out.p; fs.H = in.H; fs.W = in.W; fs.C = in.C; fs.st = st16;
    plan.resize(n - 3);
    plan.push_back(fs);
}

static Tens add_stem_pool(apse_ctx* c, const Tens& cur) {
    Step st; st.kind = S_MAXPOOL; st.x = cur.p; st.H = cur.H; st.W = cur.W; st.C = cur.C;
    Tens o = make_t(c, "stem", c->cfg.max_batch, (cur.H + 2 - 3) / 2 + 1, (cur.W + 2 - 3) / 2 + 1, cur.C, cur.st);
    st.y = o.p; st.c.name = "stem.pool"; st.st = cur.st;
    c->backbone.push_back(st);
    return o;
}

static int add_mask_predictor(apse_ctx* c, const Tens& in, Tens* logits) {
    const int KD = c->cfg.dets_per_image;
    Tens md;
    ConvSpec dc{"mask_deconv", {"roi_heads.mask_head.deconv"}, 1, 1, 1, 0, 1};
    dc.deconv = 1; dc.items = KD; dc.count_kind = 2;
    int rc = add_conv(c, c->maskhead, dc, in, &md);
    if (rc) return rc;
    ConvSpec ml{"mask_logits", {"roi_heads.mask_head.predictor"}, 1, 1, 1, 0, 0};
    ml.items = KD; ml.count_kind = 2;
    return add_conv(c, c->maskhead, ml, md, logits);
}

static int add_box_predictor(apse_ctx* c, const Tens& in) {
    ConvSpec sp{"box_pred", {"roi_heads.box_predictor.cls_score", "roi_heads.box_predictor.bbox_pred"}, 1, 1, 1, 0, 0};
    sp.items = c->cfg.rpn_post_topk; sp.count_kind = 1;
    sp.y_ld = c->pred_ld = apse_roundup(5 * c->cfg.num_classes + 1, 32);
    Tens pr;
    int rc = add_conv(c, c->boxhead, sp, in, &pr);
    if (rc) return rc;
    if (pr.C != c->pred_ld || c->t["box_pred"].st != 0) return fail(c, APSE_E_INVALID, "fused box predictor layout");
    return APSE_OK;
}

int build_plan(apse_ctx* c) {
    const apse_config& g = c->cfg;
    const int B = g.max_batch;
    c->PH = apse_roundup(g.image_h, 32);
    c->PW = apse_roundup(g.image_w, 32);
    layout_results(c);
    c->res = dalloc<uint8_t>(c, c->lay.bytes);
    if (!c->res) return fail(c, APSE_E_NOMEM, "results alloc");
    int rc;
    Tens cur;
    bool fused_stem = false;
    if (storage_type(c)) {
        Tens x0 = make_t(c, "input", B, c->PH / 2, c->PW / 2, 16, storage_type(c));
        ConvSpec sp{"stem.conv1", {"backbone.bottom_up.stem.conv1"}, 4, 4, 1, 2, 1};
        sp.s2d = 1;
        if (!getenv("APSE_NO_STEM_FUSE")) {
            Tens pooled = make_t(c, "stem", B, (x0.H + 2 - 3) / 2 + 1, (x0.W + 2 - 3) / 2 + 1, 64, storage_type(c));
            if (!pooled.p) return fail(c, APSE_E_NOMEM, "stem alloc");
            Tens unused;
            sp.out_view = &pooled;
            rc = add_conv(c, c->backbone, sp, x0, &unused);
            if (rc) return rc;
            c->t.erase("stem.conv1");
            c->backbone.back().c.pool_y = pooled.p;
            cur = pooled;
            fused_stem = true;
        } else {
            rc = add_conv(c, c->backbone, sp, x0, &cur);
        }
    } else {
        Tens x0 = make_t(c, "input", B, c->PH, c->PW, 4);
        rc = add_conv(c, c->backbone, ConvSpec{"stem.conv1", {"backbone.bottom_up.stem.conv1"}, 7, 7, 2, 3, 1}, x0, &cur);
    }
    if (rc) return rc;
    if (!fused_stem) cur = add_stem_pool(c, cur);
    for (int si = 0; si < 4; ++si) {
        const std::string stage = "res" + std::to_string(si + 2);
        for (int bi = 0; bi < g.blocks[si]; ++bi) {
            const std::string P = "backbone.bottom_up." + stage + "." + std::to_string(bi);
            const int stride = (bi == 0 && si > 0) ? 2 : 1;
            const bool last = (bi == g.blocks[si] - 1);
            Tens out;
            rc = add_bottleneck(c, c->backbone, P, P, cur, 1, stride, 0, last ? stage : P + ".out", &out);
            if (rc) return rc;
            fuse_bottleneck16(c, c->backbone, P + ".fused", cur, out);
            cur = out;
        }
    }
    Tens inner, pl[5];
    for (int lvl = 5; lvl >= 2; --lvl) {
        char ln[64], on[64], rn[16], in_name[16], pn[8];
        snprintf(ln, sizeof ln, "backbone.fpn_lateral%d", lvl);
        snprintf(on, sizeof on, "backbone.fpn_output%d", lvl);
        snprintf(rn, sizeof rn, "res%d", lvl);
        snprintf(in_name, sizeof in_name, "inner%d", lvl);
        snprintf(pn, sizeof pn, "p%d", lvl);
        Tens ninner;
        ConvSpec lat{ln, {ln}, 1, 1, 1, 0, 0};
        lat.out_name = in_name;
        if (lvl != 5) { lat.res = &inner; lat.res_mode = 2; }
        rc = add_conv(c, c->backbone, lat, c->t[rn], &ninner);
        if (rc) return rc;
        inner = ninner;
        ConvSpec outc{on, {on}, 3, 3, 1, 1, 0};
        outc.out_name = pn;
        rc = add_conv(c, c->backbone, outc, inner, &pl[lvl - 2]);
        if (rc) return rc;
    }
    {
        Step st; st.kind = S_SUBSAMPLE; st.x = pl[3].p; st.H = pl[3].H; st.W = pl[3].W; st.C = 256;
        pl[4] = make_t(c, "p6", B, (pl[3].H - 1) / 2 + 1, (pl[3].W - 1) / 2 + 1, 256, pl[3].st);
        st.y = pl[4].p; st.c.name = "p6"; st.st = pl[3].st;
        c->backbone.push_back(st);
    }
    static const int sizes[5] = {32, 64, 128, 256, 512};
    static const int strides[5] = {4, 8, 16, 32, 64};
    memset(&c->rl_host, 0, sizeof(c->rl_host));
    c->rl_host.head_ld = 16;
    c->rl_host.pre_topk = g.rpn_pre_topk;
    size_t rows_total = 0, row_off[6] = {0};
    for (int l = 0; l < 5; ++l) { row_off[l] = rows_total; rows_total += (size_t)B * pl[l].H * pl[l].W; }
    row_off[5] = rows_total;
    const int rpn_st = storage_type(c);
    Tens t_all = make_t(c, "rpn_t_all", 1, 1, (int)rows_total, 256, rpn_st);
    if (!t_all.p) return fail(c, APSE_E_NOMEM, "rpn feature buffer");
    for (int l = 0; l < 5; ++l) {
        char tn[32];
        snprintf(tn, sizeof tn, "rpn_t%d", l + 2);
        Tens view = t_all;
        view.p = reinterpret_cast<float*>(reinterpret_cast<char*>(t_all.p) + row_off[l] * 256 * (rpn_st ? 2 : 4));
        Tens tt;
        ConvSpec sp{tn, {"proposal_generator.rpn_head.conv"}, 3, 3, 1, 1, 1};
        sp.out_view = &view;
        rc = add_conv(c, c->rpnhead, sp, pl[l], &tt);
        if (rc) return rc;
    }
    Tens h_all;
    {
        Tens in_all = t_all;
        float* hbuf = dalloc<float>(c, rows_total * 16);
        if (!hbuf) return fail(c, APSE_E_NOMEM, "rpn head buffer");
        ConvSpec sp{"rpn_head_all", {"proposal_generator.rpn_head.objectness_logits", "proposal_generator.rpn_head.anchor_deltas"},
                    1, 1, 1, 0, 0};
        sp.y_ld = 16; sp.out_ptr = hbuf;
        rc = add_conv(c, c->rpnhead, sp, in_all, &h_all);
        if (rc) return rc;
        ConvStep& hs = c->rpnhead.back().c;
        hs.fixed_items = 1;
        hs.flops_per_item /= (double)B;
    }
    for (int l = 0; l < 5; ++l) {
        char hn[32];
        snprintf(hn, sizeof hn, "rpn_head%d", l + 2);
        Tens hh = h_all;
        hh.p = h_all.p + row_off[l] * 16;
        hh.H = pl[l].H; hh.W = pl[l].W; hh.C = 16;
        c->t[hn] = hh;
        RpnLevel& L = c->rl_host.lv[l];
        L.head = hh.p; L.H = hh.H; L.W = hh.W; L.stride = strides[l];
        L.n = hh.H * hh.W * 3;
        L.k = L.n < g.rpn_pre_topk ? L.n : g.rpn_pre_topk;
        static const double ratios[3] = {0.5, 1.0, 2.0};
        for (int a = 0; a < 3; ++a) {
            const double area = (double)sizes[l] * sizes[l];
            const double w = sqrt(area / ratios[a]), h = ratios[a] * w;
            L.base[a][0] = (float)(-w / 2.0); L.base[a][1] = (float)(-h / 2.0);
            L.base[a][2] = (float)(w / 2.0); L.base[a][3] = (float)(h / 2.0);
        }
    }
    c->rl_dev = dalloc<RpnLevels>(c, 1);
    hipMemcpy(c->rl_dev, &c->rl_host, sizeof(RpnLevels), hipMemcpyHostToDevice);
    {
        int slot = 0;
        std::vector<std::vector<int>> cur_slots(5), cur_counts(5);
        std::vector<TopkJob> st0;
        for (int l = 0; l < 5; ++l) {
            const int n = c->rl_host.lv[l].n;
            for (int beg = 0; beg < n; beg += 4096) {
                TopkJob j; memset(&j, 0, sizeof j);
                j.kind = 0; j.level = l; j.begin = beg; j.count = (n - beg) < 4096 ? (n - beg) : 4096;
                j.dst = slot++; j.dst_count = j.count < g.rpn_pre_topk ? j.count : g.rpn_pre_topk;
                cur_slots[l].push_back(j.dst); cur_counts[l].push_back(j.dst_count);
                st0.push_back(j);
            }
        }
        c->stages.push_back(st0);
        for (;;) {
            std::vector<TopkJob> stn;
            bool any = false;
            for (int l = 0; l < 5; ++l) {
                if (cur_slots[l].size() <= 1) continue;
                any = true;
                std::vector<int> ns, nc;
                for (size_t i = 0; i < cur_slots[l].size(); i += 4) {
                    TopkJob j; memset(&j, 0, sizeof j);
                    j.kind = 1; j.level = l; int tot = 0;
                    for (size_t k = i; k < i + 4 && k < cur_slots[l].size(); ++k) {
                        j.src[j.nsrc] = cur_slots[l][k]; j.src_count[j.nsrc] = cur_counts[l][k]; tot += cur_counts[l][k]; ++j.nsrc;
                    }
                    j.dst = slot++; j.dst_count = tot < g.rpn_pre_topk ? tot : g.rpn_pre_topk;
                    ns.push_back(j.dst); nc.push_back(j.dst_count);
                    stn.push_back(j);
                }
                cur_slots[l] = ns; cur_counts[l] = nc;
            }
            if (!any) break;
            c->stages.push_back(stn);
        }
        c->nslots = slot;
        for (int l = 0; l < 5; ++l) c->final_slot_host[l] = cur_slots[l][0];
        for (auto& sv : c->stages) c->stage_dev.push_back(dupload(c, sv));
        std::vector<int> fs(c->final_slot_host, c->final_slot_host + 5);
        c->final_slot_dev = dupload(c, fs);
        c->lists = dalloc<uint64_t>(c, (size_t)B * slot * 1024);
    }
    if ((rc = alloc_proposals(c, 5))) return rc;
    const int POST = g.rpn_post_topk, KD = g.dets_per_image;
    for (int l = 0; l < 4; ++l) { c->fm.p[l] = pl[l].p; c->fm.H[l] = pl[l].H; c->fm.W[l] = pl[l].W; c->fm.scale[l] = 1.0f / (float)strides[l]; }
    c->fm.st = pl[0].st;
    Tens pooled = make_t(c, "box_pooled", B * POST, 7, 7, 256, storage_type(c));
    Tens f1, f2;
    ConvSpec fc1{"box_fc1", {"roi_heads.box_head.fc1"}, 7, 7, 1, 0, 1, 7, 7};
    fc1.items = POST; fc1.count_kind = 1;
    rc = add_conv(c, c->boxhead, fc1, pooled, &f1);
    if (rc) return rc;
    ConvSpec fc2{"box_fc2", {"roi_heads.box_head.fc2"}, 1, 1, 1, 0, 1};
    fc2.items = POST; fc2.count_kind = 1;
    rc = add_conv(c, c->boxhead, fc2, f1, &f2);
    if (rc) return rc;
    if ((rc = add_box_predictor(c, f2))) return rc;
    alloc_box_inference(c);
    const int NM = B * KD;
    Tens mp = make_t(c, "mask_pooled", NM, 14, 14, 256, storage_type(c));
    Tens m = mp, ml;
    for (int i = 1; i <= 4; ++i) {
        char nm[48], wn[64];
        snprintf(nm, sizeof nm, "mask_fcn%d", i);
        snprintf(wn, sizeof wn, "roi_heads.mask_head.mask_fcn%d", i);
        Tens o;
        ConvSpec sp{nm, {wn}, 3, 3, 1, 1, 1};
        sp.items = KD; sp.count_kind = 2;
        rc = add_conv(c, c->maskhead, sp, m, &o);
        if (rc) return rc;
        m = o;
    }
    if ((rc = add_mask_predictor(c, m, &ml))) return rc;
    return finish_plan(c, 256);
}

static int add_res5(apse_ctx* c, std::vector<Step>& plan, const Tens& in, int items, int count_kind, const std::string& tag, Tens* out) {
    Tens cur = in;
    for (int bi = 0; bi < c->cfg.blocks[3]; ++bi) {
        const std::string T = tag + "." + std::to_string(bi);
        Tens o;
        int rc = add_bottleneck(c, plan, "roi_heads.res5." + std::to_string(bi), T, cur, items, bi == 0 ? 2 : 1, count_kind,
                                T + ".out" + std::to_string(bi), &o);
        if (rc) return rc;
        cur = o;
    }
    *out = cur;
    return APSE_OK;
}

int build_plan_c4(apse_ctx* c) {
    const apse_config& g = c->cfg;
    const int B = g.max_batch;
    c->PH = g.image_h;
    c->PW = g.image_w;
    layout_results(c);
    c->res = dalloc<uint8_t>(c, c->lay.bytes);
    if (!c->res) return fail(c, APSE_E_NOMEM, "results alloc");
    int rc;
    Tens cur;
    Tens x0 = make_t(c, "input", B, c->PH, c->PW, 4);
    rc = add_conv(c, c->backbone, ConvSpec{"stem.conv1", {"backbone.stem.conv1"}, 7, 7, 2, 3, 1}, x0, &cur);
    if (rc) return rc;
    cur = add_stem_pool(c, cur);
    for (int si = 0; si < 3; ++si) {
        const std::string stage = "res" + std::to_string(si + 2);
        for (int bi = 0; bi < g.blocks[si]; ++bi) {
            const std::string P = "backbone." + stage + "." + std::to_string(bi);
            const int stride = (bi == 0 && si > 0) ? 2 : 1;
            const bool last = bi == g.blocks[si] - 1;
            Tens out;
            rc = add_bottleneck(c, c->backbone, P, P, cur, 1, stride, 0, last ? stage : P + ".out", &out);
            if (rc) return rc;
            cur = out;
        }
    }
    const Tens res4 = c->t["res4"];
    if (res4.C < 256 || (res4.C & 255)) return fail(c, APSE_E_INVALID, "C4: res4 needs a multiple of 256 channels");
    {
        Tens t, h;
        rc = add_conv(c, c->rpnhead, ConvSpec{"rpn_conv", {"proposal_generator.rpn_head.conv"}, 3, 3, 1, 1, 1}, res4, &t);
        if (rc) return rc;
        ConvSpec sp{"rpn_head", {"proposal_generator.rpn_head.objectness_logits", "proposal_generator.rpn_head.anchor_deltas"},
                    1, 1, 1, 0, 0};
        sp.y_ld = 80;
        rc = add_conv(c, c->rpnhead, sp, t, &h);
        if (rc) return rc;
        if (c->rpnhead.back().c.p.Cout != 75) return fail(c, APSE_E_INVALID, "C4 RPN head: expected 15 objectness + 60 delta channels");
        C4Rpn& R = c->c4r;
        memset(&R, 0, sizeof R);
        R.head = h.p; R.H = h.H; R.W = h.W; R.ld = 80; R.stride = 16;
        R.n = h.H * h.W * 15;
        R.k = R.n < g.rpn_pre_topk ? R.n : g.rpn_pre_topk;
        static const int sizes[5] = {32, 64, 128, 256, 512};
        static const double ratios[3] = {0.5, 1.0, 2.0};
        for (int si = 0; si < 5; ++si)
            for (int a = 0; a < 3; ++a) {
                const double area = (double)sizes[si] * sizes[si];
                const double w = sqrt(area / ratios[a]), hh = ratios[a] * w;
                float* bb = R.base[3 * si + a];
                bb[0] = (float)(-w / 2.0); bb[1] = (float)(-hh / 2.0); bb[2] = (float)(w / 2.0); bb[3] = (float)(hh / 2.0);
            }
    }
    if ((rc = alloc_proposals(c, 1))) return rc;
    const int POST = g.rpn_post_topk, KD = g.dets_per_image;
    Tens pooled = make_t(c, "box_pooled", B * POST, 14, 14, res4.C);
    if (!pooled.p) return fail(c, APSE_E_NOMEM, "C4 box features");
    Tens r5;
    rc = add_res5(c, c->c4_res5box, pooled, POST, 1, "box_res5", &r5);
    if (rc) return rc;
    c->t["box_res5"] = r5;
    Tens mean = make_t(c, "box_mean", B * POST, 1, 1, r5.C);
    if ((rc = add_box_predictor(c, mean))) return rc;
    alloc_box_inference(c);
    const int NM = B * KD;
    Tens mp = make_t(c, "mask_pooled", NM, 14, 14, res4.C);
    Tens m5, ml;
    rc = add_res5(c, c->maskhead, mp, KD, 2, "mask_res5", &m5);
    if (rc) return rc;
    if ((rc = add_mask_predictor(c, m5, &ml))) return rc;
    if (ml.H != 14 || ml.W != 14) return fail(c, APSE_E_INVALID, "C4 mask logits must be 14 x 14");
    return finish_plan(c, res4.C);
}
```

apse_uav_amd/networks/track_rcnn.py:

```python
import collections
import ctypes as C

import numpy as np
import torch

from .. import _lib
from ..structures.instances import Boxes, Instances
from ..structures.window_mask import MaskList, WindowMask
from ..utils import resample
from ..config import check_c4_supported, is_c4
from ..weights import blocks_from_state, is_c4_state


class _Shape:
    def __init__(self, channels, stride):
        self.channels, self.stride = channels, stride


class _Backbone:

    def __init__(self, c4=False):
        self.c4 = c4
        self.size_divisibility = 0 if c4 else 32

    def output_shape(self):
        if self.c4:
            return {"res4": _Shape(1024, 16)}
        return {"p%d" % l: _Shape(256, 2 ** l) for l in range(2, 7)}


def c4_res4_size(image_h, image_w):
    h, w = image_h, image_w
    for _ in range(4):
        h, w = (h - 1) // 2 + 1, (w - 1) // 2 + 1
    return h, w


class LazyFeatures(dict):

    def __init__(self, model, batch):
        super().__init__()
        self._model, self._batch = model, batch

    def __missing__(self, key):
        if self._model.backbone.c4 and key not in self.keys():
            raise KeyError(key)
        t = self._model.export_feature(key, self._batch)
        self[key] = t
        return t

    def keys(self):
        return ["res4"] if self._model.backbone.c4 else ["p2", "p3", "p4", "p5", "p6"]


class FrameResults:

    def __init__(self, raw, lay, batch):
        self.raw, self.lay, self.batch = raw, lay, batch
        n, kd, e = lay.n_max, lay.dets_per_image, lay.embed_dim

        def arr(off, dtype, shape):
            cnt = int(np.prod(shape))
            return np.frombuffer(raw, dtype=dtype, count=cnt, offset=off).reshape(shape)

        self.total = int(arr(lay.total, np.int32, (1,))[0])
        self.offset = arr(lay.offset, np.int32, (lay.max_batch + 1,))
        self.prop_count = arr(lay.prop_count, np.int32, (lay.max_batch,))
        self.img = arr(lay.img, np.int32, (n,))
        self.cls = arr(lay.cls, np.int32, (n,))
        self.roi = arr(lay.roi, np.int32, (n,))
        self.score = arr(lay.score, np.float32, (n,))
        self.box_resized = arr(lay.box_resized, np.float32, (n, 4))
        self.box = arr(lay.box, np.float32, (n, 4))
        self.valid = arr(lay.valid, np.int32, (n,))
        self.rect = arr(lay.rect, np.int32, (n, 4))
        self.mass = arr(lay.mass, np.int32, (n,))
        self.centroid = arr(lay.centroid, np.int32, (n, 2))
        self.closest = arr(lay.closest, np.int32, (n, kd, 2))
        self.embedding = arr(lay.embedding, np.float32, (n, e))

    def image_slice(self, b):
        return int(self.offset[b]), int(self.offset[b + 1])

    def record(self, b):
        lo, hi = self.image_slice(b)
        keep = np.nonzero(self.valid[lo:hi])[0]
        idx = lo + keep
        return dict(
            boxes=self.box[idx].copy(), scores=self.score[idx].copy(), classes=self.cls[idx].astype(np.int64),
            centroids=self.centroid[idx].copy(), mass=self.mass[idx].copy(), rects=self.rect[idx].copy(),
            closest=self.closest[idx][:, keep, :].copy(), embeddings=self.embedding[idx].copy(), packed_index=idx.copy())


class TrackRCNN:
    def __init__(self, cfg):
        self.cfg = cfg
        self.device = torch.device(cfg.MODEL.DEVICE)
        self.c4 = is_c4(cfg)
        if self.c4:
            check_c4_supported(cfg)
        self.backbone = _Backbone(self.c4)
        self.training = False
        self._state = None
        self._assoc = None
        self._ctx = None
        self._ctx_key = None
        self._cache = collections.OrderedDict()
        self.contexts_built = 0
        self._lay = None
        self._host = None
        self._camera = None
        self._input_tag = None
        self._running_tag = None
        self.last_results = None

    def to(self, device):
        self.device = torch.device(device)
        return self

    def eval(self):
        self.training = False
        return self

    def load_state_dict(self, sd):
        self._state = {k: v.detach().to(torch.float32).cpu().contiguous() for k, v in sd.items()}
        self._drop_ctx()

    def attach_association_head(self, head):
        self._assoc = head
        self._drop_ctx()

    def set_camera(self, preproc):
        self._camera = preproc
        for entry in self._cache.values():
            self._push_camera(entry[0])

    def _push_camera(self, ctx):
        lib = _lib.load()
        pc = self._camera
        if pc is None:
            _lib.check(lib.apse_set_camera(ctx, None, None, 0, None, 0, 0), ctx, "apse_set_camera")
            return
        _lib.check(lib.apse_set_camera(ctx, pc.mtx.ctypes.data_as(C.POINTER(C.c_double)), pc.dist.ctypes.data_as(C.POINTER(C.c_double)),
                                       int(pc.dist.size), _lib.ptr(pc.lut_host), int(pc.undistort), int(pc.gamma_correct)),
                   ctx, "apse_set_camera")

    def _drop_ctx(self):
        self._input_tag = None
        self._running_tag = None
        self._ctx = None
        self._ctx_key = None
        while self._cache:
            _, entry = self._cache.popitem(last=False)
            _lib.load().apse_destroy(entry[0])

    def __del__(self):
        try:
            self._drop_ctx()
        except Exception:
            pass

    def _ensure_ctx(self, frame_hw, image_hw):
        key = (tuple(frame_hw), tuple(image_hw))
        if self._ctx is not None and self._ctx_key == key:
            return
        keep = int(self.cfg.APSE.get("CONTEXT_CACHE", 1))
        if keep <= 1:
            self._drop_ctx()
        else:
            self._input_tag = None
            self._running_tag = None
            if key in self._cache:
                self._cache.move_to_end(key)
                self._ctx, self._lay, self._host, self._cfg_c = self._cache[key]
                self._ctx_key = key
                return
            self._ctx = None
            self._ctx_key = None
            while len(self._cache) >= keep:
                _, entry = self._cache.popitem(last=False)
                _lib.load().apse_destroy(entry[0])
        if self.device.type != "cuda" or not torch.cuda.is_available():
            raise _lib.ApseError("the apse_uav hot path needs a ROCm GPU (cfg.MODEL.DEVICE=%s): no CPU fallback" % self.device)
        if self._state is None:
            raise _lib.ApseError("no detector weights loaded")
        if is_c4_state(self._state) != self.c4:
            raise _lib.ApseError("the detector weights are a %s checkpoint but the config is %s (MODEL.ROI_HEADS.NAME = %s)"
                                 % ("C4" if is_c4_state(self._state) else "FPN", "C4" if self.c4 else "FPN",
                                    self.cfg.MODEL.ROI_HEADS.NAME))
        lib = _lib.load()
        cfg = self.cfg
        c = _lib.ConfigArch()
        c.struct_size = C.sizeof(_lib.ConfigArch)
        c.device = self.device.index if self.device.index is not None else torch.cuda.current_device()
        c.max_batch = int(cfg.APSE.MAX_BATCH)
        c.frame_h, c.frame_w = int(frame_hw[0]), int(frame_hw[1])
        c.image_h, c.image_w = int(image_hw[0]), int(image_hw[1])
        blocks = blocks_from_state(self._state)
        for i in range(4):
            c.blocks[i] = blocks[i]
        c.num_classes = int(cfg.MODEL.ROI_HEADS.NUM_CLASSES)
        c.score_thresh = float(cfg.MODEL.ROI_HEADS.SCORE_THRESH_TEST)
        c.box_nms = float(cfg.MODEL.ROI_HEADS.NMS_THRESH_TEST)
        c.rpn_nms = float(cfg.MODEL.RPN.NMS_THRESH)
        c.mask_thresh = 0.5
        c.rpn_pre_topk = int(cfg.MODEL.RPN.PRE_NMS_TOPK_TEST)
        c.rpn_post_topk = int(cfg.MODEL.RPN.POST_NMS_TOPK_TEST)
        c.dets_per_image = int(cfg.TEST.DETECTIONS_PER_IMAGE)
        for i in range(3):
            c.pixel_mean[i] = float(cfg.MODEL.PIXEL_MEAN[i])
        roi = self._assoc.roi_size if self._assoc is not None else 10
        c.assoc_roi = roi
        c.embed_dim = self._assoc.embedding_dim if self._assoc is not None else 128
        ph = (c.image_h + 31) // 32 * 32
        pw = (c.image_w + 31) // 32 * 32
        c.assoc_scale = (pw // 4) / float(c.frame_w)
        depth = 256
        c.arch = 0
        if self.c4:
            c.arch = 1
            depth = 1024
            c.assoc_scale = c4_res4_size(c.image_h, c.image_w)[1] / float(c.frame_w)
        c.compute_dtype = {"f32": 0, "bf16": 1, "f16": 2, "fp16": 2}[str(cfg.APSE.DTYPE)]
        c.storage16 = int(bool(cfg.APSE.get("STORAGE16", True))) if c.compute_dtype else 0
        ctx = C.c_void_p()
        _lib.check(lib.apse_create(C.byref(c), C.byref(ctx)), None, "apse_create: " + lib.apse_last_error(None).decode())
        try:
            sd = dict(self._state)
            if self._assoc is not None:
                sd["association.fc.weight"] = self._assoc.fc.weight
                sd["association.fc.bias"] = self._assoc.fc.bias
            else:
                sd["association.fc.weight"] = torch.zeros(c.embed_dim, depth * roi * roi)
                sd["association.fc.bias"] = torch.zeros(c.embed_dim)
            for name, t in sd.items():
                if name.startswith("proposal_generator.anchor_generator") or name in ("pixel_mean", "pixel_std"):
                    continue
                a = np.ascontiguousarray(t.numpy(), dtype=np.float32)
                shp = (C.c_int64 * a.ndim)(*a.shape)
                _lib.check(lib.apse_set_weight(ctx, name.encode(), _lib.ptr(a), shp, a.ndim), ctx, "apse_set_weight")
            _lib.check(lib.apse_finalize_weights(ctx), ctx, "apse_finalize_weights")
            hb, hc, hk = resample.precompute_coeffs(c.frame_w, c.image_w)
            vb, vc, vk = resample.precompute_coeffs(c.frame_h, c.image_h)
            _lib.check(lib.apse_set_resize_tables(ctx, _lib.ptr(hb), _lib.ptr(hc), hk, _lib.ptr(vb), _lib.ptr(vc), vk), ctx,
                       "apse_set_resize_tables")
            lay = _lib.ResultsLayout()
            _lib.check(lib.apse_results_describe(ctx, C.byref(lay)), ctx, "apse_results_describe")
        except Exception:
            lib.apse_destroy(ctx)
            raise
        self._ctx, self._ctx_key, self._lay = ctx, key, lay
        self.contexts_built += 1
        self._host = torch.empty(lay.bytes, dtype=torch.uint8).pin_memory()
        self._cfg_c = c
        self._cache[key] = (ctx, lay, self._host, c)
        if self._camera is not None:
            self._push_camera(ctx)

    def _call(self, fn, *args):
        lib = _lib.load()
        _lib.check(getattr(lib, fn)(self._ctx, *args), self._ctx, fn)

    def preprocess_frames(self, frames, tag=None):
        B, H, W, _ = frames.shape
        ih, iw = resample.resize_shortest_edge(H, W, self.cfg.INPUT.MIN_SIZE_TEST, self.cfg.INPUT.MAX_SIZE_TEST)
        self._ensure_ctx((H, W), (ih, iw))
        self._input_tag = None
        self._running_tag = None
        self._call("apse_preprocess_frames", _lib.ptr(frames.contiguous()), B, _lib.stream_ptr())
        self._input_tag = tag
        return B

    def preprocess_images(self, images, frame_hw):
        B, _, h, w = images.shape
        self._ensure_ctx(frame_hw, (h, w))
        self._input_tag = None
        self._running_tag = None
        self._call("apse_preprocess_images", _lib.ptr(images.contiguous()), B, _lib.stream_ptr())
        return B

    def run(self, batch, given=None, rpn_levels=31):
        self._running_tag = None
        s = _lib.stream_ptr()
        self._call("apse_backbone", batch, s)
        if given is None:
            self._call("apse_rpn_levels", batch, int(rpn_levels), s)
            self._call("apse_box_head", batch, s)
        else:
            boxes, classes, counts = given
            boxes = np.ascontiguousarray(boxes, np.float32).reshape(-1, 4)
            classes = np.ascontiguousarray(classes, np.int32)
            counts = np.ascontiguousarray(counts, np.int32)
            self._call("apse_set_detections", _lib.ptr(boxes), _lib.ptr(classes), None, _lib.ptr(counts), batch, s)
        self._call("apse_mask_tail", batch, s)
        self._call("apse_embed", batch, s)

    def read(self, batch):
        self.read_begin(batch)
        return self.read_end(batch)

    def read_begin(self, batch):
        self._call("apse_read_results_begin", C.c_void_p(self._host.data_ptr()), self._lay.bytes, _lib.stream_ptr())

    def read_end(self, batch):
        self._call("apse_read_results_end", C.c_void_p(self._host.data_ptr()))
        raw = self._host.numpy().tobytes()
        self.last_results = FrameResults(raw, self._lay, batch)
        return self.last_results

    def export_feature(self, name, batch):
        shp = (C.c_int * 3)()
        self._call("apse_feature_shape", name.encode(), C.byref(shp))
        out = torch.empty((batch, shp[0], shp[1], shp[2]), dtype=torch.float32, device=self.device)
        self._call("apse_export_feature", name.encode(), _lib.ptr(out), batch, _lib.stream_ptr())
        return out

    def debug_tensor(self, name, dtype=torch.float32):
        n = C.c_size_t()
        self._call("apse_debug_tensor", name.encode(), None, 0, C.byref(n), _lib.stream_ptr())
        out = torch.empty(n.value // torch.empty((), dtype=dtype).element_size(), dtype=dtype, device=self.device)
        self._call("apse_debug_tensor", name.encode(), _lib.ptr(out), n.value, C.byref(n), _lib.stream_ptr())
        return out

    def backbone_frames(self, frames):
        B = self.preprocess_frames(frames)
        self._running_tag = None
        self._call("apse_backbone", B, _lib.stream_ptr())
        return B

    def backbone_images(self, images, frame_hw):
        B = self.preprocess_images(images, frame_hw)
        self._call("apse_backbone", B, _lib.stream_ptr())
        return B

    def mask_roi_features(self, boxes, image=0):
        if self.c4:
            raise NotImplementedError("mask_roi_features pools p2..p5: not available for C4 (Res5ROIHeads) models")
        b = torch.as_tensor(boxes, dtype=torch.float32).reshape(-1, 4).to(self.device).contiguous()
        out = torch.empty((b.shape[0], 14, 14, 256), dtype=torch.float32, device=self.device)
        self._call("apse_mask_roi_features", int(image), _lib.ptr(b), b.shape[0], _lib.ptr(out), _lib.stream_ptr())
        return out

    def flops(self, batch, proposals, detections):
        return float(_lib.load().apse_flops(self._ctx, batch, proposals, detections))

    def instances_from(self, res, b, want_masks=True):
        frame_hw = self._ctx_key[0]
        rec = res.record(b)
        n = len(rec["scores"])
        inst = Instances(frame_hw)
        inst.pred_boxes = Boxes(torch.from_numpy(rec["boxes"]))
        inst.scores = torch.from_numpy(rec["scores"])
        inst.pred_classes = torch.from_numpy(rec["classes"])
        masks = MaskList()
        lib = _lib.load()
        rects = np.ascontiguousarray(rec["rects"], np.int32).reshape(n, 4)
        live = [k for k in range(n) if want_masks and rects[k, 2] > rects[k, 0] and rects[k, 3] > rects[k, 1]]
        pool, offs = None, {}
        if live:
            nw = ((rects[live, 2] + 63) >> 6) - (rects[live, 0] >> 6)
            words = nw.astype(np.int64) * (rects[live, 3] - rects[live, 1])
            off = np.zeros(len(live) + 1, np.int64)
            np.cumsum(words, out=off[1:])
            pool = torch.empty((int(off[-1]),), dtype=torch.int64, device=self.device)
            dets = np.ascontiguousarray(rec["packed_index"][live], np.int32)
            lrects = np.ascontiguousarray(rects[live])
            _lib.check(lib.apse_copy_mask_windows(self._ctx, len(live), _lib.ptr(dets), _lib.ptr(lrects), _lib.ptr(pool),
                                                  _lib.ptr(np.ascontiguousarray(off[:-1])), _lib.stream_ptr()), self._ctx, "apse_copy_mask_windows")
            offs = {k: (int(off[j]), int(off[j + 1]), int(nw[j])) for j, k in enumerate(live)}
        for k in range(n):
            x0, y0, x1, y1 = [int(v) for v in rects[k]]
            bits = None
            if k in offs:
                lo, hi, w = offs[k]
                bits = pool[lo:hi].view(y1 - y0, w)
            masks.append(WindowMask(bits, (x0, y0, x1, y1), frame_hw, rec["centroids"][k], rec["mass"][k]))
        inst.pred_masks = masks
        inst._record = rec
        return inst

    def _inference_images(self, batched_inputs, detected_instances, do_postprocess, rpn_levels):
        assert not self.training
        if not do_postprocess:
            raise NotImplementedError("do_postprocess=False is not on the CSV path and is not provided")
        B = len(batched_inputs)
        imgs = torch.stack([bi["image"].to(torch.float32) for bi in batched_inputs]).to(self.device)
        frame_hw = (int(batched_inputs[0]["height"]), int(batched_inputs[0]["width"]))
        self.preprocess_images(imgs, frame_hw)
        given = None
        if detected_instances is not None:
            assert len(detected_instances) == B
            boxes = np.concatenate([d.pred_boxes.tensor.cpu().numpy().reshape(-1, 4) for d in detected_instances])
            classes = np.concatenate([np.asarray(d.pred_classes.cpu()).reshape(-1) for d in detected_instances])
            counts = np.asarray([len(d) for d in detected_instances], np.int32)
            given = (boxes, classes, counts)
        self.run(B, given, rpn_levels)
        res = self.read(B)
        return [{"instances": self.instances_from(res, b)} for b in range(B)], B

    def inference(self, batched_inputs, detected_instances=None, do_postprocess=True):
        out, B = self._inference_images(batched_inputs, detected_instances, do_postprocess, 31)
        return out, LazyFeatures(self, B)

    def inference_frames(self, frames, given=None, want_masks=True, rpn_levels=31):
        B = self.preprocess_frames(frames)
        self.run(B, given, rpn_levels)
        res = self.read(B)
        return [self.instances_from(res, b, want_masks) for b in range(B)], LazyFeatures(self, B)
```

include/apse_hip.h:

```cpp
#ifndef APSE_HIP_H
#define APSE_HIP_H
#include <stddef.h>
#include <stdint.h>
#ifdef __cplusplus
extern "C" {
#endif

#define APSE_OK 0
#define APSE_E_INVALID (-1)
#define APSE_E_HIP (-2)
#define APSE_E_NOMEM (-3)
#define APSE_E_STATE (-4)
#define APSE_E_MISSING (-5)

typedef struct apse_ctx apse_ctx;

#define APSE_MAX_CLASSES 80
#define APSE_C4_MAX_PRE_TOPK 6000
#define APSE_C4_MAX_BATCH 2
#define APSE_MAX_FRAME_W 49152
#define APSE_MAX_FRAME_H 32768
typedef struct apse_config {
    int struct_size;
    int device;
    int max_batch;
    int frame_h, frame_w;
    int image_h, image_w;
    int blocks[4];
    int num_classes;
    float score_thresh;
    float box_nms;
    float rpn_nms;
    float mask_thresh;
    int rpn_pre_topk;
    int rpn_post_topk;
    int dets_per_image;
    float pixel_mean[3];
    int assoc_roi;
    int embed_dim;
    float assoc_scale;
    int compute_dtype;
    int storage16;
    int arch;
} apse_config;

typedef struct apse_results_layout {
    size_t bytes;
    int n_max, dets_per_image, embed_dim, max_batch;
    size_t total;
    size_t offset;
    size_t prop_count;
    size_t img;
    size_t cls;
    size_t roi;
    size_t score;
    size_t box_resized;
    size_t box;
    size_t valid;
    size_t rect;
    size_t mass;
    size_t centroid;
    size_t closest;
    size_t embedding;
} apse_results_layout;

int apse_create(const apse_config* cfg, apse_ctx** out);
void apse_destroy(apse_ctx* ctx);
const char* apse_last_error(apse_ctx* ctx);
const char* apse_version(void);

int apse_set_weight(apse_ctx* ctx, const char* name, const float* host, const int64_t* shape, int ndim);
int apse_finalize_weights(apse_ctx* ctx);

int apse_set_resize_tables(apse_ctx* ctx, const int* hbounds, const int* hcoef, int hksize, const int* vbounds,
                           const int* vcoef, int vksize);

int apse_set_camera(apse_ctx* ctx, const double* m9, const double* dist, int ndist, const uint8_t* lut256_host, int do_undistort,
                    int do_gamma);

int apse_preprocess_frames(apse_ctx* ctx, const uint8_t* frames_dev, int batch, void* stream);
int apse_preprocess_images(apse_ctx* ctx, const float* images_dev, int batch, void* stream);
int apse_backbone(apse_ctx* ctx, int batch, void* stream);
int apse_rpn(apse_ctx* ctx, int batch, void* stream);
int apse_rpn_levels(apse_ctx* ctx, int batch, int level_mask, void* stream);
int apse_box_head(apse_ctx* ctx, int batch, void* stream);
int apse_set_detections(apse_ctx* ctx, const float* boxes_host, const int* classes_host, const float* scores_host,
                        const int* counts_host, int batch, void* stream);
int apse_mask_tail(apse_ctx* ctx, int batch, void* stream);
int apse_embed(apse_ctx* ctx, int batch, void* stream);
int apse_roi_features(apse_ctx* ctx, int image, const float* rois_dev, const uint8_t* masks_dev, int n, int roi_size,
                      float* out_dev, void* stream);
int apse_forward(apse_ctx* ctx, int batch, void* stream);

int apse_results_describe(apse_ctx* ctx, apse_results_layout* out);
int apse_read_results(apse_ctx* ctx, void* host_dst, size_t bytes, void* stream);
int apse_read_results_begin(apse_ctx* ctx, void* host_dst, size_t bytes, void* stream);
int apse_read_results_end(apse_ctx* ctx, void* host_dst);
int apse_copy_mask_window(apse_ctx* ctx, int det, int x0, int y0, int x1, int y1, uint64_t* dst_dev, void* stream);
int apse_copy_mask_windows(apse_ctx* ctx, int n, const int* dets_host, const int* rects_host, uint64_t* dst_dev,
                           const long long* dst_word_offsets_host, void* stream);
int apse_feature_shape(apse_ctx* ctx, const char* name, int* chw3);
int apse_export_feature(apse_ctx* ctx, const char* name, float* dst_nchw_dev, int batch, void* stream);
int apse_debug_tensor(apse_ctx* ctx, const char* name, void* dst_dev, size_t max_bytes, size_t* bytes, void* stream);
double apse_flops(apse_ctx* ctx, int batch, double proposals, double detections);

int apse_profile(apse_ctx* ctx, int enable);
int apse_profile_read(apse_ctx* ctx, double* out42, int reset);

typedef struct apse_conv_desc {
    int B, H, W, Cin;
    int Cout, KH, KW, stride, pad;
    int relu;
    int res_mode;
    int cfg;
    int splitk;
    int prec;
    int fuse_reduce;
    int x_st, res_st, y_st;
} apse_conv_desc;
size_t apse_conv_packed_elems(const apse_conv_desc* d);
int apse_conv_pack_weight(const apse_conv_desc* d, const float* w_oihw, int cin_real, const float* scale, float* packed);
int apse_conv2d(const apse_conv_desc* d, const float* x_dev, const float* w_packed_dev, const float* bias_dev,
                const float* res_dev, float* y_dev, float* ws_dev, size_t ws_bytes, void* stream);
int apse_winograd_pack_filter(const float* w_oihw, int Cout, int Cin, float* packed);
int apse_winograd_conv2d(const apse_conv_desc* d, const float* x_dev, const float* wu_dev, const float* bias_dev, float* y_dev,
                         void* stream);
int apse_maxpool3x3s2(const float* x_dev, float* y_dev, int B, int H, int W, int C, void* stream);
int apse_maxpool3x3s2_typed(const void* x_dev, void* y_dev, int B, int H, int W, int C, int storage, void* stream);
int apse_roi_align(const float* const* feats_dev, const int* hs, const int* ws, const float* rois_dev, int n, int per_img,
                   int out_size, float* out_dev, void* stream);
int apse_roi_align_typed(const void* const* feats_dev, const int* hs, const int* ws, const float* rois_dev, int n, int per_img,
                         int out_size, int storage, void* out_dev, void* stream);
int apse_roi_pool(const float* feat_dev, int H, int W, const float* rois_dev, const int* roi_img_dev, int n, int out_size,
                  float scale, float* out_dev, void* stream);
int apse_nms_rank(const float* boxes_dev, const float* scores_dev, const int* valid_dev, int n, int cat_div, int cat_mod,
                  int ncat, float thr, int topk, float* out_boxes_dev, float* out_scores_dev, int* out_index_dev,
                  int* out_count_dev, void* stream);
int apse_mask_centroid_dense(const uint8_t* mask_dev, int H, int W, int* out_xy_mass_host3, void* stream);
int apse_mask_closest_dense(const uint8_t* mask_dev, int H, int W, float px, float py, int* out_xy_host2, void* stream);
int apse_l2_normalize(const float* x_dev, float* y_dev, int n, int D, void* stream);
int apse_sqdist(const float* a_dev, const float* b_dev, int O, int N, int D, float* out_dev, void* stream);
int apse_undistort_gamma(const uint8_t* src_dev, uint8_t* dst_dev, int B, int H, int W, const double* mtx3x3_host,
                         const double* dist_host, int ndist, const uint8_t* lut256_host, int do_undistort, int do_gamma,
                         void* stream);
size_t apse_lab_tables_host(const uint8_t* lut256_host, void* out, size_t cap);
int apse_resize_normalize(const uint8_t* frames_dev, uint8_t* tmp_dev, float* out_nhwc4_dev, uint8_t* resized_u8_dev,
                          const int* hb_dev, const int* hc_dev, int hk, const int* vb_dev, const int* vc_dev, int vk, int B,
                          int H, int W, int OH, int OW, int PH, int PW, const float* mean3_host, void* stream);

typedef struct apse_replay apse_replay;
apse_replay* apse_replay_create(int host_id, int embed_dim, float dist_thresh, int max_unseen_frames);
void apse_replay_destroy(apse_replay* r);
int apse_replay_step(apse_replay* r, int frame_idx, int n, const float* emb_host, const int* centroid_host,
                     const int* closest_host, char* line_out, int line_cap, int* det_ids_out);
long long apse_replay_packed(apse_replay* r, const float* records_host, long long total_floats, int nrec, int dets_per_image,
                             int first_frame, char* lines_out, long long cap);
int apse_replay_max_id(const apse_replay* r);
int apse_replay_next_id(const apse_replay* r);


int apse_host_copy(void* dst, const void* src, size_t bytes, int threads);

#define APSE_RENDER_MAX_ITEMS 1024
#define APSE_RENDER_MAX_BREAKS 64
#define APSE_RENDER_MAX_LINES 4
typedef struct apse_render_item {
    int image;
    int rect[4];
    int words_per_row;
    const uint64_t* bits;
    float box[4];
    uint8_t rgb[4];
    int label_off, label_len;
} apse_render_item;
size_t apse_render_workspace_bytes(int H, int W, int n);
int apse_render_instances(const uint8_t* frames_dev, uint8_t* out_dev, int B, int H, int W, int bgr,
                          const apse_render_item* items_dev, int n, const uint8_t* labels_dev, size_t label_bytes,
                          const float* scale_breaks_host, int nbreaks, void* ws_dev, size_t ws_bytes, void* stream);
int apse_render_pack_mask(const uint8_t* mask_dev, int H, int W, uint64_t* words_dev, void* stream);
size_t apse_render_font_host(uint8_t* out, size_t cap);

#define APSE_MOTS_MAX_OBJECTS 1024
#define APSE_MOTS_MAX_PAIRS 65536
#define APSE_MOTS_MAX_UNION 1024
typedef struct apse_mots_window {
    int rect[4];
    int words_per_row;
    int area;
    uint64_t* bits;
} apse_mots_window;
typedef struct apse_mots_object {
    int rect[4];
    int words_per_row;
    float score;
    const uint64_t* bits;
} apse_mots_object;
size_t apse_mots_split_workspace_bytes(void);
int apse_mots_split_idmap(const uint16_t* idmap, int H, int W, int max_values, uint64_t* pool, size_t pool_words, int* values,
                          apse_mots_window* windows, int* info, void* ws, size_t ws_bytes, void* stream);
int apse_mots_rle_to_bits(const int* ends, const int* ends_off, int n, int h, int w, const apse_mots_window* windows,
                          void* stream);
int apse_mots_overlaps(const apse_mots_window* windows, int n_windows, const int* pairs, int npairs, const int* union_idx,
                       int n_union, int* out, void* stream);
int apse_mots_shift_overlaps(const apse_mots_window* windows, int n_windows, const int* quads, int npairs, int H, int W,
                             int* out, void* stream);
int apse_mots_render_idmap(const apse_mots_object* objects, const int* values_host, int n, int H, int W, uint16_t* idmap,
                           void* stream);

#define APSE_COCO_MAX_GROUPS (1 << 24)
#define APSE_COCO_MAX_GT 4096
#define APSE_COCO_MAX_DET 4096
#define APSE_COCO_MAX_T 64
#define APSE_COCO_MAX_R 1024
#define APSE_COCO_MAX_A 16
#define APSE_COCO_MAX_M 16
#define APSE_COCO_MAX_CATS 1024
#define APSE_COCO_MAX_KEYS (1 << 24)
#define APSE_COCO_MAX_POLY_OBJECTS (1 << 20)
#define APSE_COCO_MAX_POLY_PARTS (1 << 22)
#define APSE_COCO_MAX_POLY_VERTS (1 << 26)
int apse_coco_box_iou(const int* dt_off, const int* gt_off, const long long* iou_off, int n_groups, int max_dt, int max_gt,
                      const double* dt_box, const double* gt_box, const int* gt_crowd, double* iou, void* stream);
int apse_coco_poly_to_bits(const double* xy, const int* part_vert_off, int n_parts, const int* obj_part_off, int n_obj,
                           const int* obj_hw, const int* obj_hw_host, const int* edge_off, int n_verts, int* toggles,
                           const apse_mots_window* windows, int* info, void* stream);
int apse_coco_match(const int* dt_off, const int* gt_off, const long long* iou_off, int n_groups, int max_dt, int max_gt,
                    const double* iou, const double* dt_area, const long long* dt_id, int n_dt, const double* gt_area,
                    const int* gt_crowd, const long long* gt_id, int n_gt, const double* area_rng_host, int A,
                    const double* iou_thrs_host, int T, long long* dt_match, unsigned char* dt_ignore, long long* gt_match,
                    unsigned char* gt_ignore, void* stream);
size_t apse_coco_accumulate_workspace_bytes(long long n_keys);
int apse_coco_sort_lists(const double* score, const int* seg_off, int n_seg, const int* seg_idx, long long n_keys, int max_seg,
                         int* sorted_idx, void* ws, size_t ws_bytes, void* stream);
int apse_coco_accumulate(const double* dt_score, const long long* dt_match, const unsigned char* dt_ignore, int n_dt,
                         const unsigned char* gt_ignore, int n_gt, const int* cat_gt_off, const int* seg_off,
                         const int* seg_idx, long long n_keys, int max_seg, const double* rec_thrs, int T, int R, int K, int A,
                         int M, double* precision, double* recall, double* scores, void* ws, size_t ws_bytes, void* stream);

#define APSE_ASSOC_MAX_N 2048
#define APSE_ASSOC_MAX_D 256
#define APSE_ASSOC_MAX_K (256 * 32 * 32)
size_t apse_assoc_fc_workspace_bytes(int n, int K, int D);
int apse_assoc_fc_forward(const float* x, const float* w, const float* b, int n, int K, int D, float* e, float* inv_norm,
                          float* ws, size_t ws_bytes, void* stream);
int apse_assoc_fc_backward(const float* x, const float* e, const float* inv_norm, const float* de, int n, int K, int D, float* dw,
                           float* db, float* ws, size_t ws_bytes, void* stream);
size_t apse_triplet_workspace_bytes(int n);
int apse_triplet_hard_forward(const double* labels, const float* e, int n, int D, float margin, int squared, float* loss,
                              void* ws, size_t ws_bytes, void* stream);
int apse_triplet_all_forward(const double* labels, const float* e, int n, int D, float margin, int squared, float* loss_frac,
                             void* ws, size_t ws_bytes, void* stream);
int apse_triplet_hard_backward(const float* e, int n, int D, int squared, const void* ws, const float* grad_loss, float* de,
                               void* stream);
int apse_triplet_all_backward(const float* e, int n, int D, int squared, const void* ws, const float* grad_loss, float* de,
                              void* stream);
int apse_sgd_step(float* p, const float* g, float* buf, long long n, float lr, float momentum, float dampening,
                  float weight_decay, int nesterov, int first_step, void* stream);

#define APSE_MASK_TRAIN_MAX_N 1024
int apse_mask_roi_features(apse_ctx* ctx, int image, const float* rois_dev, int n, float* out_dev, void* stream);
size_t apse_mask_train_workspace_bytes(int n, int K);
size_t apse_mask_pack_elems(int Cout, int Cin, int KH, int KW);
int apse_mask_pack_weight(const float* w_dev, const float* bias_dev, int kind, int Cout, int Cin, int KH, int KW, float* packed_dev,
                          float* bias_packed_dev, void* stream);
int apse_mask_conv_forward(const float* x_dev, const float* w_packed_dev, const float* bias_packed_dev, int n, int H, int W, int Cin,
                           int Cout, int KH, int KW, int stride, int pad, int relu, int deconv, float* y_dev, float* ws,
                           size_t ws_bytes, void* stream);
int apse_mask_conv3x3(const float* x_dev, const float* w_packed_dev, const float* bias_packed_dev, int n, int relu, float* y_dev,
                      void* stream);
int apse_mask_relu_grad(const float* y_dev, const float* dy_dev, long long elems, float* g_dev, void* stream);
int apse_mask_bias_grad(const float* g_dev, long long rows, float* db_dev, float* ws, size_t ws_bytes, void* stream);
int apse_mask_wgrad(const float* a_dev, const float* b_dev, int n, int kind, float* dw_dev, float* ws, size_t ws_bytes, void* stream);
int apse_mask_loss_forward(const float* logits_dev, int K, const int* classes_dev, const uint8_t* targets_dev, int n, float* out4_dev,
                           void* ws, size_t ws_bytes, void* stream);
int apse_mask_loss_backward(const float* logits_dev, int K, const int* classes_dev, const uint8_t* targets_dev, int n,
                            const float* grad_loss_dev, float* d_dev, void* stream);
int apse_mask_predictor_backward(const float* d_dev, const float* a5_dev, const int* classes_dev, const float* w_pred_dev, int n, int K,
                                 float* g5_dev, float* dw_dev, float* db_dev, float* ws, size_t ws_bytes, void* stream);

#define APSE_AUGMENT_MAX_BATCH 64
typedef struct { int flip; double brightness, saturation, contrast; double lighting_vec[3]; } apse_augment_params;
int apse_augment_u8(const uint8_t* src_dev, int B, int H, int W, const apse_augment_params* params_host,
                    uint8_t* out_u8_dev, float* out_chw_dev, unsigned long long* sums_dev, void* stream);

#ifdef __cplusplus
}
#endif
#endif
```

Before: 194.4.

## Run detection tail on a side stream overlapping next frame's backbone

Adds a second non-blocking HIP stream (tail lane) that runs the RPN proposal stage, box head, mask tail, embedding and result readback. While a previous read is pending, the next frame's backbone can then overlap the previous frame's tail on the caller stream. Events handle fork/join: the FPN step waits on the tail, mask-window copies wait on per-buffer bits events, and a separate split-K workspace is allocated for the lane. This adds synchronization complexity, extra memory, and a risk of hazards on shared buffers such as FPN features and the results buffer.

Result: faster. 202.5, median of 6 (+4.2%).

```diff
diff --git a/apse_uav_amd/_lib.py b/apse_uav_amd/_lib.py
--- a/apse_uav_amd/_lib.py
+++ b/apse_uav_amd/_lib.py
@@ -6,7 +6,7 @@
 _HERE = os.path.dirname(os.path.abspath(__file__))
 _TREE_LIB = os.path.join(_HERE, "libapse_hip.so")
 LIB_PATH = os.environ.get("APSE_HIP_LIB") or _TREE_LIB
-TOOL_ENTRIES = ("apse_winograd_pack_filter", "apse_winograd_conv2d")
+TOOL_ENTRIES = ("apse_winograd_pack_filter", "apse_winograd_conv2d", "apse_lane_stats")
 
 APSE_OK = 0
 
@@ -29,6 +29,10 @@
 
 class ConfigArch(Config):
     _fields_ = [("arch", C.c_int)]
+
+
+class ConfigLane(ConfigArch):
+    _fields_ = [("tail_lane", C.c_int)]
 
 
 class ResultsLayout(C.Structure):
@@ -92,6 +96,7 @@
         "apse_read_results": ([vp, vp, sz, vp], i),
         "apse_read_results_begin": ([vp, vp, sz, vp], i),
         "apse_read_results_end": ([vp, vp], i),
+        "apse_lane_stats": ([vp, C.POINTER(C.c_longlong * 4)], i),
         "apse_copy_mask_window": ([vp, i, i, i, i, i, vp, vp], i),
         "apse_copy_mask_windows": ([vp, i, vp, vp, vp, vp, vp], i),
         "apse_host_copy": ([vp, vp, sz, i], i),
@@ -179,7 +184,7 @@
 EXPORTS = ["apse_create", "apse_destroy", "apse_last_error", "apse_version", "apse_set_weight", "apse_finalize_weights",
            "apse_set_resize_tables", "apse_set_camera", "apse_preprocess_frames", "apse_preprocess_images", "apse_backbone", "apse_rpn", "apse_rpn_levels",
            "apse_box_head", "apse_set_detections", "apse_mask_tail", "apse_embed", "apse_forward", "apse_results_describe",
-           "apse_read_results", "apse_read_results_begin", "apse_read_results_end", "apse_copy_mask_window", "apse_copy_mask_windows", "apse_host_copy", "apse_feature_shape", "apse_export_feature", "apse_debug_tensor",
+           "apse_read_results", "apse_read_results_begin", "apse_read_results_end", "apse_lane_stats", "apse_copy_mask_window", "apse_copy_mask_windows", "apse_host_copy", "apse_feature_shape", "apse_export_feature", "apse_debug_tensor",
            "apse_flops", "apse_profile", "apse_profile_read", "apse_conv_packed_elems", "apse_conv_pack_weight", "apse_conv2d", "apse_winograd_pack_filter", "apse_winograd_conv2d", "apse_maxpool3x3s2",
            "apse_maxpool3x3s2_typed", "apse_roi_align", "apse_roi_align_typed", "apse_roi_pool", "apse_roi_features", "apse_nms_rank", "apse_mask_centroid_dense", "apse_mask_closest_dense",
            "apse_l2_normalize", "apse_sqdist", "apse_undistort_gamma", "apse_lab_tables_host", "apse_resize_normalize", "apse_replay_create", "apse_replay_destroy",
diff --git a/apse_uav_amd/config.py b/apse_uav_amd/config.py
--- a/apse_uav_amd/config.py
+++ b/apse_uav_amd/config.py
@@ -116,7 +116,7 @@
                   "MIN_SIZE_TRAIN_SAMPLING": "choice"},
         "TEST": {"DETECTIONS_PER_IMAGE": 100},
         "DATASETS": {"TRAIN": ("coco_2017_train",), "TEST": ("coco_2017_val",)},
-        "APSE": {"DTYPE": "f32", "MAX_BATCH": 1, "FUSED_PREPROC": True, "STORAGE16": True, "CONTEXT_CACHE": 1},
+        "APSE": {"DTYPE": "f32", "MAX_BATCH": 1, "FUSED_PREPROC": True, "STORAGE16": True, "CONTEXT_CACHE": 1, "TAIL_LANE": True},
     })
 
 
diff --git a/apse_uav_amd/csrc/detector.hip b/apse_uav_amd/csrc/detector.hip
--- a/apse_uav_amd/csrc/detector.hip
+++ b/apse_uav_amd/csrc/detector.hip
@@ -24,12 +24,98 @@
     return e0;
 }
 
+static bool lane_active(const apse_ctx* c) { return c->lane_on && !c->prof_on && c->lane_armed; }
+
+static void lane_teardown(apse_ctx* c) {
+    hipEvent_t* evs[5] = {&c->fork_ev, &c->follow_ev, &c->tail_ev, &c->bits_ev[0], &c->bits_ev[1]};
+    for (hipEvent_t* e : evs) { if (*e) hipEventDestroy(*e); *e = nullptr; }
+    if (c->lane) hipStreamDestroy(c->lane);
+    c->lane = nullptr;
+    c->fork_pending = c->follow_pending = c->tail_live = c->bits_live[0] = c->bits_live[1] = false;
+    c->caller_dirty = true;
+}
+
+static int lane_create(apse_ctx* c) {
+    if (c->lane) return APSE_OK;
+    hipEvent_t* evs[5] = {&c->fork_ev, &c->follow_ev, &c->tail_ev, &c->bits_ev[0], &c->bits_ev[1]};
+    hipError_t e = hipSuccess;
+    for (hipEvent_t* ev : evs) if (e == hipSuccess) e = hipEventCreateWithFlags(ev, hipEventDisableTiming);
+    if (e == hipSuccess) e = hipStreamCreateWithFlags(&c->lane, hipStreamNonBlocking);
+    if (e != hipSuccess) {
+        lane_teardown(c);
+        return fail(c, APSE_E_HIP, std::string("tail lane: ") + hipGetErrorString(e));
+    }
+    return APSE_OK;
+}
+
+static bool event_done(hipEvent_t ev) {
+    if (hipEventQuery(ev) == hipSuccess) return true;
+    if (hipPeekAtLastError() == hipErrorNotReady) (void)hipGetLastError();
+    return false;
+}
+
+struct LaneScope {
+    apse_ctx* c = nullptr; hipStream_t s = nullptr; bool on = false;
+    int bits_k = -1;
+    int begin(apse_ctx* c_, hipStream_t caller) {
+        c = c_; s = caller;
+        if (!lane_active(c)) return APSE_OK;
+        int rc = lane_create(c);
+        if (rc) return rc;
+        if (c->caller_dirty) {
+            HIPCHK(c, hipEventRecord(c->fork_ev, caller));
+            c->caller_dirty = false; c->fork_pending = true;
+        }
+        if (c->fork_pending) { HIPCHK(c, hipStreamWaitEvent(c->lane, c->fork_ev, 0)); c->fork_pending = false; }
+        if (c->follow_pending) { HIPCHK(c, hipStreamWaitEvent(c->lane, c->follow_ev, 0)); c->follow_pending = false; }
+        s = c->lane; on = true;
+        return APSE_OK;
+    }
+    ~LaneScope() {
+        if (!on) return;
+        if (bits_k >= 0 && hipEventRecord(c->bits_ev[bits_k], c->lane) == hipSuccess) c->bits_live[bits_k] = true;
+        if (hipEventRecord(c->tail_ev, c->lane) == hipSuccess) c->tail_live = true;
+    }
+};
+
+static int lane_join(apse_ctx* c, hipStream_t s, hipEvent_t ev, bool live) {
+    if (!c->lane || !live || event_done(ev)) return APSE_OK;
+    HIPCHK(c, hipStreamWaitEvent(s, ev, 0));
+    ++c->lane_stats[1];
+    return APSE_OK;
+}
+static int lane_join(apse_ctx* c, hipStream_t s) { return lane_join(c, s, c->tail_ev, c->tail_live); }
+static int lane_follow(apse_ctx* c, hipStream_t s) {
+    if (!c->lane) return APSE_OK;
+    HIPCHK(c, hipEventRecord(c->follow_ev, s));
+    c->follow_pending = true;
+    return APSE_OK;
+}
+static int lane_drain(apse_ctx* c) {
+    if (!c->lane) return APSE_OK;
+    if (c->tail_live && !event_done(c->tail_ev)) ++c->lane_stats[1];
+    HIPCHK(c, hipStreamSynchronize(c->lane));
+    ++c->lane_stats[3];
+    return APSE_OK;
+}
+
+static void count_lane_forward(apse_ctx* c, bool on) {
+    if (!on || c->fwd_counted) return;
+    ++c->lane_stats[0];
+    c->fwd_counted = true;
+}
+
 static int run_plan(apse_ctx* c, std::vector<Step>& plan, int batch, hipStream_t s) {
     int* total_dev = reinterpret_cast<int*>(c->res + c->lay.total);
     int* propcnt_dev = reinterpret_cast<int*>(c->res + c->lay.prop_count);
+    float* ws = (c->lane && s == c->lane) ? c->ws_lane : c->ws;
     for (size_t si = 0; si < plan.size(); ++si) {
         Step& st = plan[si];
         int rc = APSE_OK;
+        if (&plan == &c->backbone && (int)si == c->fpn_step && c->lane && c->tail_live && !event_done(c->tail_ev)) {
+            ++c->lane_stats[2];
+            HIPCHK(c, hipStreamWaitEvent(s, c->tail_ev, 0));
+        }
         if (st.kind == S_CONV) {
             ConvParams p = st.c.p;
             for (size_t sj = si + 1; sj < plan.size() && sj <= si + 2; ++sj)
@@ -43,7 +129,7 @@
                 }
             p.B = st.c.fixed_items > 0 ? st.c.fixed_items : batch * st.c.b_mult;
             p.M = p.B * p.OH * p.OW;
-            p.ws = c->ws;
+            p.ws = ws;
             p.tile_cnt = nullptr;
             p.m_count = nullptr; p.m_per_item = p.OH * p.OW; p.m_hint = 0;
             int cfg = st.c.cfg;
@@ -113,8 +199,8 @@
 
 int apse_create(const apse_config* cfg, apse_ctx** out) {
     if (!cfg || !out) return fail(nullptr, APSE_E_INVALID, "null argument");
-    const int old_size = (int)offsetof(apse_config, arch);
-    if (cfg->struct_size != (int)sizeof(apse_config) && cfg->struct_size != old_size)
+    const int old_size = (int)offsetof(apse_config, arch), arch_size = (int)offsetof(apse_config, tail_lane);
+    if (cfg->struct_size != (int)sizeof(apse_config) && cfg->struct_size != old_size && cfg->struct_size != arch_size)
         return fail(nullptr, APSE_E_INVALID, "apse_config size mismatch");
     apse_config cf;
     memset(&cf, 0, sizeof cf);
@@ -163,6 +249,10 @@
         const char* e = getenv("APSE_F32_WINOGRAD");
         c->f32_winograd = !(e && atoi(e) == 0);
     }
+    {
+        const char* e = getenv("APSE_TAIL_LANE");
+        c->lane_on = !c->c4 && cfg->tail_lane >= 0 && !(e && atoi(e) == 0);
+    }
     *out = c;
     return APSE_OK;
 }
@@ -170,6 +260,10 @@
 void apse_destroy(apse_ctx* c) {
     if (!c) return;
     hipSetDevice(c->cfg.device);
+    if (c->lane) {
+        hipStreamSynchronize(c->lane);
+        lane_teardown(c);
+    }
     for (void* p : c->allocs) hipFree(p);
     if (c->rf_mask) hipFree(c->rf_mask);
     if (c->mrf_idx) hipFree(c->mrf_idx);
@@ -250,6 +344,10 @@
 
 int apse_backbone(apse_ctx* c, int batch, void* stream) {
     NEED_READY(c, batch);
+    c->caller_dirty = true;
+    c->lane_armed = c->read_pending != nullptr;
+    c->fwd_since_read = true;
+    c->fwd_counted = false;
     return run_plan(c, c->backbone, batch, (hipStream_t)stream);
 }
 
@@ -262,8 +360,15 @@
     hipStream_t s = (hipStream_t)stream;
     const apse_config& g = c->cfg;
     if (c->c4 && level_mask != 31) return fail(c, APSE_E_INVALID, "C4 (arch 1) has one RPN level: level_mask must be 31");
-    int rc = run_plan(c, c->rpnhead, batch, s);
-    if (rc) return rc;
+    int rc;
+    if (!c->caller_dirty && (rc = lane_join(c, s))) return rc;
+    rc = run_plan(c, c->rpnhead, batch, s);
+    if (rc) return rc;
+    c->caller_dirty = true;
+    LaneScope ln;
+    if ((rc = ln.begin(c, s))) return rc;
+    count_lane_forward(c, ln.on);
+    s = ln.s;
     if (c->c4) {
         int* propcnt = reinterpret_cast<int*>(c->res + c->lay.prop_count);
         rc = apse_k_c4_rpn(&c->c4r, g.rpn_pre_topk, g.rpn_post_topk, (float)g.image_h, (float)g.image_w, (float)log(1000.0 / 16.0),
@@ -305,11 +410,13 @@
 
 int apse_box_head(apse_ctx* c, int batch, void* stream) {
     NEED_READY(c, batch);
-    hipStream_t s = (hipStream_t)stream;
+    LaneScope ln;
+    int rc = ln.begin(c, (hipStream_t)stream);
+    if (rc) return rc;
+    hipStream_t s = ln.s;
     const apse_config& g = c->cfg;
     int* propcnt = reinterpret_cast<int*>(c->res + c->lay.prop_count);
     const int P = g.rpn_post_topk, K = g.num_classes;
-    int rc;
     if (c->c4) {
         const Tens& f = c->t["res4"];
         rc = apse_k_roi_align_c4(f.p, f.H, f.W, f.C, 1.0f / 16.0f, c->props, nullptr, propcnt, nullptr, P, batch * P, 14,
@@ -361,7 +468,11 @@
 int apse_set_detections(apse_ctx* c, const float* boxes, const int* classes, const float* scores, const int* counts, int batch,
                         void* stream) {
     NEED_READY(c, batch);
-    hipStream_t s = (hipStream_t)stream;
+    LaneScope ln;
+    int rc = ln.begin(c, (hipStream_t)stream);
+    if (rc) return rc;
+    count_lane_forward(c, ln.on);
+    hipStream_t s = ln.s;
     const apse_config& g = c->cfg;
     const int KD = g.dets_per_image, K = g.num_classes;
     const size_t nb = (size_t)g.max_batch * KD;
@@ -397,18 +508,20 @@
     HIPCHK(c, hipMemcpyAsync(c->det_entry, de, nbb * 4, hipMemcpyHostToDevice, s));
     HIPCHK(c, hipMemcpyAsync(c->det_cnt, dc, (size_t)batch * 4, hipMemcpyHostToDevice, s));
     HIPCHK(c, hipEventRecord(c->given_ev[slot], s));
-    int rc = pack_from_dets(c, batch, s);
+    rc = pack_from_dets(c, batch, s);
     return rc ? fail(c, rc, "pack launch failed") : APSE_OK;
 }
 
 int apse_mask_tail(apse_ctx* c, int batch, void* stream) {
     NEED_READY(c, batch);
-    hipStream_t s = (hipStream_t)stream;
+    LaneScope ln;
+    int rc = ln.begin(c, (hipStream_t)stream);
+    if (rc) return rc;
+    hipStream_t s = ln.s;
     const apse_config& g = c->cfg;
     uint8_t* r = c->res;
     const int NM = batch * g.dets_per_image;
     int* total = (int*)(r + c->lay.total);
-    int rc;
     if (c->c4) {
         const Tens& f = c->t["res4"];
         rc = apse_k_roi_align_c4(f.p, f.H, f.W, f.C, 1.0f / 16.0f, (float*)(r + c->lay.box_resized), (int*)(r + c->lay.img), nullptr,
@@ -429,6 +542,7 @@
     if (c->sums_dirty) HIPCHK(c, hipMemsetAsync(c->sums, 0, (size_t)g.max_batch * g.dets_per_image * 3 * sizeof(unsigned long long), s));
     c->sums_dirty = true;
     c->bits_cur ^= 1;
+    ln.bits_k = c->bits_cur;
     if (!c->read_pending) c->bits_read = c->bits_cur;
     uint64_t* bits = c->bits2[c->bits_cur];
     p.bits = bits; p.sums = c->sums;
@@ -443,12 +557,14 @@
 
 int apse_embed(apse_ctx* c, int batch, void* stream) {
     NEED_READY(c, batch);
-    hipStream_t s = (hipStream_t)stream;
+    LaneScope ln;
+    int rc = ln.begin(c, (hipStream_t)stream);
+    if (rc) return rc;
+    hipStream_t s = ln.s;
     const apse_config& g = c->cfg;
     uint8_t* r = c->res;
     const int NM = batch * g.dets_per_image;
     int* total = (int*)(r + c->lay.total);
-    int rc;
     if (c->c4) {
         const Tens& f = c->t["res4"];
         rc = apse_k_roi_pool_c4(f.p, f.H, f.W, f.C, (float*)(r + c->lay.box), (int*)(r + c->lay.img), total, NM, g.assoc_roi,
@@ -490,9 +606,13 @@
     if (!c || !c->finalized) return fail(c, APSE_E_STATE, "not finalized");
     if (bytes < c->lay.bytes) return fail(c, APSE_E_INVALID, "results buffer too small");
     if (!c->read_ev) HIPCHK(c, hipEventCreateWithFlags(&c->read_ev, hipEventDisableTiming));
-    HIPCHK(c, hipMemcpyAsync(host_dst, c->res, c->lay.bytes, hipMemcpyDeviceToHost, (hipStream_t)stream));
-    HIPCHK(c, hipEventRecord(c->read_ev, (hipStream_t)stream));
+    LaneScope ln;
+    int rc = ln.begin(c, (hipStream_t)stream);
+    if (rc) return rc;
+    HIPCHK(c, hipMemcpyAsync(host_dst, c->res, c->lay.bytes, hipMemcpyDeviceToHost, ln.s));
+    HIPCHK(c, hipEventRecord(c->read_ev, ln.s));
     c->read_pending = host_dst;
+    c->fwd_since_read = false;
     c->bits_read = c->bits_cur;
     if (c->prof_on) {
         c->pending_read.swap(c->pending);
@@ -509,6 +629,11 @@
     if (!c->read_pending || c->read_pending != host_dst) return fail(c, APSE_E_STATE, "apse_read_results_end without a matching _begin");
     HIPCHK(c, hipEventSynchronize(c->read_ev));
     c->read_pending = nullptr;
+    if (c->lane && !c->fwd_since_read && !c->prof_on) {
+        HIPCHK(c, hipStreamSynchronize(c->lane));
+        lane_teardown(c);
+        ++c->lane_stats[3];
+    }
     c->hint_total = *reinterpret_cast<const int*>(reinterpret_cast<const uint8_t*>(host_dst) + c->lay.total);
     {
         uint8_t* h = reinterpret_cast<uint8_t*>(host_dst) + c->lay.closest;
@@ -554,6 +679,9 @@
 
 int apse_profile(apse_ctx* c, int enable) {
     if (!c) return APSE_E_INVALID;
+    int rc = lane_drain(c);
+    if (rc) return rc;
+    c->caller_dirty = true;
     if (enable && c->ev_pool.empty()) {
         c->ev_pool.resize(2 * APSE_EV_HALF);
         for (auto& e : c->ev_pool) if (hipEventCreate(&e) != hipSuccess) return fail(c, APSE_E_HIP, "hipEventCreate");
@@ -566,6 +694,12 @@
     return APSE_OK;
 }
 
+int apse_lane_stats(apse_ctx* c, long long* out4) {
+    if (!c || !out4) return APSE_E_INVALID;
+    memcpy(out4, c->lane_stats, sizeof(c->lane_stats));
+    return APSE_OK;
+}
+
 int apse_profile_read(apse_ctx* c, double* out42, int reset) {
     if (!c || !out42) return APSE_E_INVALID;
     memcpy(out42, c->prof, sizeof(c->prof));
@@ -580,9 +714,11 @@
         return fail(c, APSE_E_INVALID, "bad mask window");
     const int w0 = x0 >> 6, w1 = (x1 + 63) >> 6;
     const uint64_t* src = c->bits2[c->bits_read] + ((size_t)det * g.frame_h + y0) * c->wpr + w0;
+    int rc = lane_join(c, (hipStream_t)stream, c->bits_ev[c->bits_read], c->bits_live[c->bits_read]);
+    if (rc) return rc;
     HIPCHK(c, hipMemcpy2DAsync(dst, (size_t)(w1 - w0) * 8, src, (size_t)c->wpr * 8, (size_t)(w1 - w0) * 8, (size_t)(y1 - y0),
                                hipMemcpyDeviceToDevice, (hipStream_t)stream));
-    return APSE_OK;
+    return lane_follow(c, (hipStream_t)stream);
 }
 
 int apse_copy_mask_windows(apse_ctx* c, int n, const int* dets, const int* rects, uint64_t* dst, const long long* dst_off, void* stream) {
@@ -599,8 +735,11 @@
         src[k] = ((long long)dets[k] * g.frame_h + y0) * c->wpr + w0;
         nw[k] = w1 - w0; rows[k] = y1 - y0;
     }
-    int rc = apse_k_copy_mask_windows(c->bits2[c->bits_read], dst, n, src, dst_off, nw, rows, c->wpr, (hipStream_t)stream);
-    return rc ? fail(c, rc, "mask windows launch failed") : APSE_OK;
+    int rc = lane_join(c, (hipStream_t)stream, c->bits_ev[c->bits_read], c->bits_live[c->bits_read]);
+    if (rc) return rc;
+    rc = apse_k_copy_mask_windows(c->bits2[c->bits_read], dst, n, src, dst_off, nw, rows, c->wpr, (hipStream_t)stream);
+    if (rc) return fail(c, rc, "mask windows launch failed");
+    return lane_follow(c, (hipStream_t)stream);
 }
 
 int apse_feature_shape(apse_ctx* c, const char* name, int* chw3) {
@@ -616,8 +755,11 @@
     auto it = c->t.find(name);
     if (it == c->t.end()) return fail(c, APSE_E_MISSING, std::string("no tensor ") + name);
     const Tens& t = it->second;
-    int rc = apse_k_nhwc_to_nchw(t.p, dst, batch, t.H * t.W, t.C, t.st, (hipStream_t)stream);
-    return rc ? fail(c, rc, "export launch failed") : APSE_OK;
+    int rc = lane_join(c, (hipStream_t)stream);
+    if (rc) return rc;
+    rc = apse_k_nhwc_to_nchw(t.p, dst, batch, t.H * t.W, t.C, t.st, (hipStream_t)stream);
+    if (rc) return fail(c, rc, "export launch failed");
+    return lane_follow(c, (hipStream_t)stream);
 }
 
 int apse_roi_features(apse_ctx* c, int image, const float* rois, const uint8_t* masks, int n, int roi_size, float* out, void* stream) {
@@ -630,7 +772,8 @@
     hipStream_t s = (hipStream_t)stream;
     const Tens& p2 = c->t["p2"];
     const float scale = (float)p2.W / (float)g.frame_w;
-    int rc;
+    int rc = lane_join(c, s);
+    if (rc) return rc;
     if (!masks) {
         rc = apse_k_roi_pool(p2.p, p2.st, p2.H, p2.W, rois, nullptr, nullptr, n, roi_size, scale, out, image, 1, s);
         return rc ? fail(c, rc, "roi_pool launch failed") : APSE_OK;
@@ -667,7 +810,9 @@
     FpnMaps fm = c->fm;
     for (int l = 0; l < 4; ++l)
         fm.p[l] = reinterpret_cast<const char*>(fm.p[l]) + (size_t)image * fm.H[l] * fm.W[l] * 256 * (fm.st ? 2 : 4);
-    int rc = apse_k_mask_roi_index(c->mrf_idx, n, s);
+    int rc = lane_join(c, s);
+    if (rc) return rc;
+    rc = apse_k_mask_roi_index(c->mrf_idx, n, s);
     if (rc) return fail(c, rc, "mask_roi_features index launch failed");
     rc = apse_k_roi_align(&fm, rois, c->mrf_idx, nullptr, c->mrf_idx + n, 0, n, 14, out, 0, s);
     return rc ? fail(c, rc, "roi_align(14) launch failed") : APSE_OK;
@@ -706,8 +851,10 @@
     if (bytes) *bytes = n;
     if (!dst) return APSE_OK;
     if (n > max_bytes) return fail(c, APSE_E_INVALID, "debug buffer too small for " + nm);
+    int rc = lane_join(c, (hipStream_t)stream);
+    if (rc) return rc;
     HIPCHK(c, hipMemcpyAsync(dst, src, n, hipMemcpyDeviceToDevice, (hipStream_t)stream));
-    return APSE_OK;
+    return lane_follow(c, (hipStream_t)stream);
 }
 
 double apse_flops(apse_ctx* c, int batch, double proposals, double detections) {
@@ -724,6 +871,7 @@
 
 int apse_set_camera(apse_ctx* c, const double* m, const double* dist, int ndist, const uint8_t* lut_host, int do_undistort, int do_gamma) {
     if (!c) return APSE_E_INVALID;
+    if (lane_drain(c)) return APSE_E_HIP;
     if (!do_undistort && !do_gamma) { c->cam_on = false; return APSE_OK; }
     if (do_gamma && !lut_host) return fail(c, APSE_E_INVALID, "gamma needs a 256-entry LUT");
     UndistortParams p;
diff --git a/apse_uav_amd/csrc/detector_ctx.h b/apse_uav_amd/csrc/detector_ctx.h
--- a/apse_uav_amd/csrc/detector_ctx.h
+++ b/apse_uav_amd/csrc/detector_ctx.h
@@ -68,6 +68,18 @@
     struct Pending { int cfg; double flops_per_item; int count_kind; int b_mult; int batch; int e0, e1; };
     std::vector<Pending> pending; double prof[APSE_NCFG][3] = {{0}};
     int ev_base = 0, cal_read = -1; std::vector<Pending> pending_read;
+    bool lane_on = true;
+    bool lane_armed = false;
+    bool fwd_since_read = false;
+    hipStream_t lane = nullptr;
+    hipEvent_t fork_ev = nullptr, follow_ev = nullptr, tail_ev = nullptr, bits_ev[2] = {nullptr, nullptr};
+    bool caller_dirty = false;
+    bool fork_pending = false, follow_pending = false;
+    bool tail_live = false, bits_live[2] = {false, false};
+    float* ws_lane = nullptr;
+    int fpn_step = -1;
+    long long lane_stats[4] = {0, 0, 0, 0};
+    bool fwd_counted = false;
     uint64_t* op_bits = nullptr; unsigned long long* op_sums = nullptr; size_t op_bits_words = 0;
     bool c4 = false;
     C4Rpn c4r; void* c4_nms = nullptr;
diff --git a/apse_uav_amd/csrc/plan.hip b/apse_uav_amd/csrc/plan.hip
--- a/apse_uav_amd/csrc/plan.hip
+++ b/apse_uav_amd/csrc/plan.hip
@@ -320,6 +320,20 @@
         c->ws = dalloc<float>(c, c->ws_floats, false);
         if (!c->ws) return fail(c, APSE_E_NOMEM, "split-K workspace alloc");
     }
+    if (c->lane_on) {
+        size_t need = 0;
+        for (const std::vector<Step>* pl : {&c->boxhead, &c->maskhead, &c->embedfc})
+            for (const Step& st : *pl) {
+                const ConvParams& q = st.c.p;
+                if (st.kind != S_CONV || q.splitk <= 1) continue;
+                const size_t n = (size_t)q.splitk * B * st.c.b_mult * q.OH * q.OW * q.Cout;
+                if (n > need) need = n;
+            }
+        if (need) {
+            c->ws_lane = dalloc<float>(c, need, false);
+            if (!c->ws_lane) return fail(c, APSE_E_NOMEM, "tail lane split-K workspace alloc");
+        }
+    }
     c->tile_cnt = dalloc<int>(c, 65536);
     c->rs_pitch = (g.image_w * 3 + 15) & ~15;
     c->rs_tmp = dalloc<uint8_t>(c, (size_t)B * g.frame_h * c->rs_pitch, false);
@@ -448,6 +462,7 @@
             cur = out;
         }
     }
+    c->fpn_step = (int)c->backbone.size();
     Tens inner, pl[5];
     for (int lvl = 5; lvl >= 2; --lvl) {
         char ln[64], on[64], rn[16], in_name[16], pn[8];
diff --git a/apse_uav_amd/networks/track_rcnn.py b/apse_uav_amd/networks/track_rcnn.py
--- a/apse_uav_amd/networks/track_rcnn.py
+++ b/apse_uav_amd/networks/track_rcnn.py
@@ -110,6 +110,7 @@
         self._lay = None
         self._host = None
         self._camera = None
+        self.tail_lane = None
         self._input_tag = None
         self._running_tag = None
         self.last_results = None
@@ -223,6 +224,12 @@
             c.assoc_scale = c4_res4_size(c.image_h, c.image_w)[1] / float(c.frame_w)
         c.compute_dtype = {"f32": 0, "bf16": 1, "f16": 2, "fp16": 2}[str(cfg.APSE.DTYPE)]
         c.storage16 = int(bool(cfg.APSE.get("STORAGE16", True))) if c.compute_dtype else 0
+        lane = bool(cfg.APSE.get("TAIL_LANE", True)) if self.tail_lane is None else bool(self.tail_lane)
+        if not lane and hasattr(lib, "apse_lane_stats"):
+            c, short = _lib.ConfigLane(), c
+            C.memmove(C.byref(c), C.byref(short), C.sizeof(_lib.ConfigArch))
+            c.struct_size = C.sizeof(_lib.ConfigLane)
+            c.tail_lane = -1
         ctx = C.c_void_p()
         _lib.check(lib.apse_create(C.byref(c), C.byref(ctx)), None, "apse_create: " + lib.apse_last_error(None).decode())
         try:
@@ -307,6 +314,11 @@
         raw = self._host.numpy().tobytes()
         self.last_results = FrameResults(raw, self._lay, batch)
         return self.last_results
+
+    def lane_stats(self):
+        out = (C.c_longlong * 4)()
+        self._call("apse_lane_stats", C.byref(out))
+        return tuple(int(v) for v in out)
 
     def export_feature(self, name, batch):
         shp = (C.c_int * 3)()
diff --git a/include/apse_hip.h b/include/apse_hip.h
--- a/include/apse_hip.h
+++ b/include/apse_hip.h
@@ -42,6 +42,7 @@
     int compute_dtype;
     int storage16;
     int arch;
+    int tail_lane;
 } apse_config;
 
 typedef struct apse_results_layout {
@@ -96,6 +97,7 @@
 int apse_read_results(apse_ctx* ctx, void* host_dst, size_t bytes, void* stream);
 int apse_read_results_begin(apse_ctx* ctx, void* host_dst, size_t bytes, void* stream);
 int apse_read_results_end(apse_ctx* ctx, void* host_dst);
+int apse_lane_stats(apse_ctx* ctx, long long* out4);
 int apse_copy_mask_window(apse_ctx* ctx, int det, int x0, int y0, int x1, int y1, uint64_t* dst_dev, void* stream);
 int apse_copy_mask_windows(apse_ctx* ctx, int n, const int* dets_host, const int* rects_host, uint64_t* dst_dev,
                            const long long* dst_word_offsets_host, void* stream);
```
